# xenji/kafka-topic-analyzer

Measured on NVIDIA H100. Metric: messages/sec scanned (fused metric scan), higher is better.
Workload: dtype u64

## Files before the change

kafka_topic_analyzer_b200/csrc/kta_api.cu:

```cuda
#include <cuda_runtime.h>

#include <algorithm>
#include <chrono>
#include <climits>
#include <cmath>
#include <cstdarg>
#include <cstdio>
#include <cstdlib>
#include <cstring>
#include <new>
#include <vector>

#include "kta_host.cuh"
#include "kta_kernels.cuh"
#include "kta_logscan.cuh"
#include "kta_partitioner.cuh"
#include "kta_synth.h"
#include "kta_timeline.cuh"

using namespace kta;

extern "C" const char *kta_last_error(void) { return g_err; }
extern "C" int kta_abi_version(void) { return KTA_ABI_VERSION; }
extern "C" int kta_device_count(void) {
    int n = 0;
    if (cudaGetDeviceCount(&n) != cudaSuccess) {
        cudaGetLastError();
        return -1;
    }
    return n;
}

static constexpr int NCHUNK = 3;
static constexpr int32_t ALIVE_DEFAULT_KIB = 256 * 1024;
static constexpr int32_t ALIVE_MAX_KIB = 32 * 1024 * 1024;
static constexpr int64_t ALIVE_CACHE_MIN_RECORDS = 1 << 20;
static constexpr int64_t DEFAULT_RING_RECORDS = 1 << 22;

struct Chunk {
    DevBuf<int32_t> d_partition, d_klen, d_vlen;
    DevBuf<int64_t> d_ts;
    DevBuf<uint64_t> d_seq;
    DevBuf<uint8_t> d_keys;
    DevBuf<uint64_t> d_tile_base;
    cudaEvent_t free_ev = nullptr;
    PinnedBuf<int32_t> h_partition, h_klen, h_vlen;
    PinnedBuf<int64_t> h_ts;
    PinnedBuf<uint8_t> h_keys;
    PinnedBuf<uint64_t> h_tile_base;
};

struct AlivePending {
    ScanParams prm;
    int64_t key_readable, key_bytes;
    int chunk;
    const uint32_t *hash; const uint64_t *stamp; int64_t count;
};

struct AliveKeys {
    DevBuf<unsigned long long> d_table;
    uint32_t pairs = 0;
    uint64_t origin = 0;
    bool rebased = false;
    DevBuf<uint32_t> d_cache;
    DevBuf<uint32_t> d_status;
    PinnedBuf<uint32_t> h_status;
    DevBuf<unsigned long long> d_count;
    uint64_t window_errors = 0;
    uint64_t grows = 0, reruns = 0;
    uint64_t now = 0, occupied = 0;
    std::vector<AlivePending> pending;
};

struct Timeline {
    int32_t buckets = 0;
    int64_t origin = 0, width = 1;
    bool smem = false;
    int blocks_per_sm = 0;
    DevBuf<unsigned long long> d_bins;
    std::vector<uint64_t> h_bins;
    size_t words() const { return d_bins.cap > 0 ? (size_t)d_bins.cap : 0; }
};

struct Partitioner {
    int32_t ncounts = 0;
    int32_t counts[KTA_PARTITIONER_MAX_COUNTS] = {};
    bool smem = false;
    int32_t max_grid = 0;
    DevBuf<unsigned long long> d_counts;
    std::vector<uint64_t> h_counts;
    size_t words() const { return d_counts.cap > 0 ? (size_t)d_counts.cap : 0; }
};

struct kta_handle {
    kta_config cfg{};
    int device = 0;
    int sm_count = 0;
    cudaStream_t stream = nullptr;
    bool own_stream = true;
    bool need_hash = false;
    DevBuf<unsigned long long> d_sums;
    DevBuf<long long> d_minmax;
    DevBuf<uint32_t> d_hll;
    DevBuf<uint32_t> d_hll_floor;
    AliveKeys alive;
    uint32_t *d_hash_out = nullptr;
    DevBuf<uint64_t> d_tb_scratch;
    LogScan log;
    Timeline tl;
    Partitioner pt;
    DevBuf<uint32_t> d_crc32_tables;
    size_t nsums = 0, nhll = 0;
    Chunk chunks[NCHUNK];
    bool ring_dev_ready = false, ring_host_ready = false;
    int64_t ring_records = 0, ring_key_bytes = 0;
    int cur = 0;
    struct PushCursor {
        int32_t *part = nullptr, *klen = nullptr, *vlen = nullptr;
        int64_t *ts = nullptr;
        uint8_t *keys = nullptr;
        uint64_t *tile_base = nullptr;
        int64_t n = 0, cap = 0;
        int64_t kb = 0, kcap = 0;
        bool hash = false;
    } pc;
    uint64_t next_seq = 0;
    bool finalized = false;
    std::vector<uint64_t> h_sums;
    long long h_minmax[4] = {0, 0, 0, 0};
    std::vector<uint32_t> h_hll;
    uint64_t h_alive = 0;
    int shard_world = 1, shard_rank = 0;
    int columns = 0;
    bool smem_counters = true;
    size_t smem_optin = 0;
    uint64_t launches = 0, records = 0;
    bool timing = false;
    std::vector<std::pair<cudaEvent_t, cudaEvent_t>> ev_pool;
    size_t ev_used = 0;
    double scan_ms = 0;
    uint64_t scan_launches_timed = 0;
};

static int set_device(const kta_handle *h) {
    CU(cudaSetDevice(h->device));
    return KTA_OK;
}

static bool keys_travel(const kta_handle *h) { return h->need_hash || h->d_hash_out || h->pt.ncounts; }

static size_t scan_smem_bytes(bool hash, bool smem, int P, int threads, int keybuf, int stages, bool hdr) {
    return (smem ? smem_counter_bytes(P) : CTA_SCRATCH) + (size_t)(threads / 32) * warp_smem_bytes(hash, keybuf, stages, hdr);
}

static void scan_shape(const kta_handle *h, bool hash, bool hdr_ok, int64_t n, int64_t key_bytes, int &threads, int &keybuf,
                       int &stages, bool &hdr, size_t &smem) {
    const int P = h->columns;
    keybuf = KEYBUF_MIN;
    stages = 0;
    hdr = false;
    if (!hash) {
        threads = MAX_THREADS;
        smem = scan_smem_bytes(false, h->smem_counters, P, threads, keybuf, stages, hdr);
        return;
    }
    if (n > 0) {
        const int64_t per_tile = (key_bytes * TILE + n - 1) / n;
        int64_t want = per_tile + per_tile / 8 + 64 + KEYBUF_SLACK;
        want = (want + 127) / 128 * 128;
        keybuf = (int)std::min<int64_t>(std::max<int64_t>(want, KEYBUF_MIN), KEYBUF_MAX);
        keybuf = (keybuf + 15) / 16 * 16;
    }
    auto fits = [&](bool with_hdr, int st, int max_warps, int min_warps) {
        hdr = with_hdr;
        stages = st;
        for (threads = std::min(max_warps * 32, HASH_MAX_THREADS); threads >= min_warps * 32; threads -= 32) {
            smem = scan_smem_bytes(true, h->smem_counters, P, threads, keybuf, stages, hdr);
            if (smem <= h->smem_optin) return true;
        }
        return false;
    };
    if (hdr_ok && (fits(true, SCAN_STAGES, 12, 10) || fits(true, 2, 12, 10))) return;
    if (fits(false, 2, 16, 8)) return;
    keybuf = KEYBUF_MIN;
    fits(false, 2, 16, 1);
}

using ScanFn = void (*)(ScanParams);
static const ScanFn SCAN_KERNELS[2][2][3][2] = {
    {{{scan_kernel<MODE_COUNTERS, false, false, false>, nullptr},
      {scan_kernel<MODE_HLL, false, false, false>, scan_kernel<MODE_HLL, false, true, false>},
      {scan_kernel<MODE_EXACT, false, false, false>, scan_kernel<MODE_EXACT, false, true, false>}},
     {{scan_kernel<MODE_COUNTERS, false, false, true>, nullptr},
      {scan_kernel<MODE_HLL, false, false, true>, nullptr},
      {scan_kernel<MODE_EXACT, false, false, true>, nullptr}}},
    {{{scan_kernel<MODE_COUNTERS, true, false, false>, nullptr},
      {scan_kernel<MODE_HLL, true, false, false>, scan_kernel<MODE_HLL, true, true, false>},
      {scan_kernel<MODE_EXACT, true, false, false>, scan_kernel<MODE_EXACT, true, true, false>}},
     {{scan_kernel<MODE_COUNTERS, true, false, true>, nullptr},
      {scan_kernel<MODE_HLL, true, false, true>, nullptr},
      {scan_kernel<MODE_EXACT, true, false, true>, nullptr}}},
};

static int launch_scan_raw(kta_handle *h, ScanParams prm, int64_t key_readable, int64_t key_bytes);
static int ring_flush(kta_handle *h);

static int alive_create(kta_handle *h) {
    const int64_t kib = h->cfg.alive_table_kib;
    if (kib < 0 || kib > ALIVE_MAX_KIB) return fail(KTA_ERR_INVALID, "alive_table_kib %d out of range [0, %d]", (int)kib, ALIVE_MAX_KIB);
    AliveKeys &a = h->alive;
    a.pairs = (uint32_t)std::max<int64_t>((kib ? kib : ALIVE_DEFAULT_KIB) * 64, 16);
    int rc;
    if ((rc = a.d_table.alloc((int64_t)a.pairs * 2)) || (rc = a.d_status.alloc(3)) || (rc = a.d_count.alloc(3)) ||
        (rc = a.d_cache.alloc((int64_t)1 << ALIVE_CACHE_SET_BITS)) || (rc = a.h_status.alloc(2 * (NCHUNK + 1))))
        return rc;
    return KTA_OK;
}

static int alive_reset(kta_handle *h) {
    AliveKeys &a = h->alive;
    if (!a.d_table) return KTA_OK;
    CU(cudaMemsetAsync(a.d_table, 0xff, (size_t)a.pairs * 16, h->stream));
    CU(cudaMemsetAsync(a.d_status, 0, 12, h->stream));
    a.now = a.occupied = a.origin = 0;
    a.rebased = false;
    a.window_errors = 0;
    a.pending.clear();
    return KTA_OK;
}

static int alive_grow(kta_handle *h, uint32_t new_pairs) {
    AliveKeys &a = h->alive;
    cudaStream_t s = h->stream;
    DevBuf<unsigned long long> nt;
    int rc;
    if ((rc = nt.alloc((int64_t)new_pairs * 2))) return rc;
    CU(cudaMemsetAsync(nt, 0xff, (size_t)new_pairs * 16, s));
    alive_rehash_kernel<<<h->sm_count * 8, THREADS, 0, s>>>(a.d_table, (size_t)a.pairs * 2, nt, new_pairs, a.d_status);
    h->launches++;
    CU(cudaGetLastError());
    CU(cudaStreamSynchronize(s));
    a.d_table = std::move(nt);
    a.pairs = new_pairs;
    a.grows++;
    return KTA_OK;
}

static int alive_apply(kta_handle *h, const AlivePending &p) {
    AliveKeys &a = h->alive;
    if (p.count) {
        const int grid = (int)std::min<int64_t>((p.count + THREADS - 1) / THREADS, (int64_t)h->sm_count * 8);
        alive_import_kernel<<<grid, THREADS, 0, h->stream>>>(AliveTable{a.d_table, a.pairs, a.d_status, 0}, a.origin, p.hash,
                                                             reinterpret_cast<const unsigned long long *>(p.stamp), p.count);
        h->launches++;
        CU(cudaGetLastError());
        return KTA_OK;
    }
    ScanParams prm = p.prm;
    prm.alive_only = 1;
    prm.alive_table = a.d_table;
    prm.alive_pairs = a.pairs;
    a.reruns++;
    return launch_scan_raw(h, prm, p.key_readable, p.key_bytes);
}

static int alive_settle(kta_handle *h) {
    AliveKeys &a = h->alive;
    if (!a.d_table) return KTA_OK;
    cudaStream_t s = h->stream;
    for (int round = 0;; round++) {
        unsigned long long counts[3] = {0, 0, 0};
        CU(cudaMemsetAsync(a.d_count, 0, 24, s));
        alive_count_kernel<<<h->sm_count * 8, THREADS, 0, s>>>(a.d_table, (size_t)a.pairs * 2, a.d_count);
        h->launches++;
        CU(cudaGetLastError());
        CU(cudaMemcpyAsync(a.h_status, a.d_status, 8, cudaMemcpyDeviceToHost, s));
        CU(cudaMemcpyAsync(counts, a.d_count, 24, cudaMemcpyDeviceToHost, s));
        CU(cudaStreamSynchronize(s));
        const unsigned long long occupied = counts[2];
        a.now = counts[0];
        a.occupied = occupied;
        const uint32_t dropped = a.h_status[0];
        a.window_errors += a.h_status[1];
        if (dropped || a.h_status[1]) CU(cudaMemsetAsync(a.d_status, 0, 8, s));
        const uint64_t slots = (uint64_t)a.pairs * 2;
        const bool crowded = occupied * 10 > slots * 6;
        if (!dropped && !crowded) break;
        const bool wide = dropped && (occupied + dropped) * 10 <= slots * 6;
        int rc;
        if (!wide) {
            if (a.pairs >= (uint32_t)ALIVE_MAX_KIB * 64u) {
                if (dropped) return fail(KTA_ERR_NOMEM, "alive-key table is at its maximum (32 GiB) and still too full");
                break;
            }
            uint64_t want = slots * 2;
            while (want < (occupied + dropped) * 2) want *= 2;
            want = std::min<uint64_t>(want, (uint64_t)ALIVE_MAX_KIB * 128ull);
            if ((rc = alive_grow(h, (uint32_t)(want / 2)))) return rc;
            if (!dropped) break;
        }
        if (round > 40) return fail(KTA_ERR_INVALID, "alive-key table growth did not converge");
        if (wide) CU(cudaMemsetAsync(a.d_status + 2, 0xff, 4, s));
        for (const AlivePending &p : a.pending)
            if ((rc = alive_apply(h, p))) return rc;
        if (wide) CU(cudaMemsetAsync(a.d_status + 2, 0, 4, s));
    }
    a.pending.clear();
    return KTA_OK;
}

static int alive_settle_if_any(kta_handle *h) { return h->alive.pending.empty() ? KTA_OK : alive_settle(h); }

static int alive_prepare(kta_handle *h, ScanParams &prm, const uint64_t *seq_ends) {
    AliveKeys &a = h->alive;
    int rc;
    if ((uint64_t)prm.n > (uint64_t)ALIVE_FIELD_MAX - 1)
        return fail(KTA_ERR_INVALID, "batch of %lld records with count_alive_keys: split it (< 2^31 per scan)", (long long)prm.n);
    if (prm.seq_base < a.origin)
        return fail(KTA_ERR_INVALID, "seq_base %llu lies before the alive-key table's window origin %llu (batches must not "
                    "go back past a rebase)", (unsigned long long)prm.seq_base, (unsigned long long)a.origin);
    if (!prm.seq && prm.seq_base - a.origin + (uint64_t)prm.n > (uint64_t)ALIVE_FIELD_MAX) {
        if ((rc = alive_settle(h))) return rc;
        if (!a.pending.empty()) return fail(KTA_ERR_INVALID, "internal: alive-key stamps pending across a rebase");
        alive_rebase_kernel<<<h->sm_count * 8, THREADS, 0, h->stream>>>(a.d_table, (size_t)a.pairs * 2);
        h->launches++;
        CU(cudaGetLastError());
        a.origin = prm.seq_base;
        a.rebased = true;
    }
    prm.alive_table = a.d_table;
    prm.alive_pairs = a.pairs;
    prm.alive_origin = a.origin;
    prm.alive_fbase = prm.seq_base - a.origin + 1ull;
    prm.alive_status = a.d_status;
    if (prm.n >= ALIVE_CACHE_MIN_RECORDS) {
        uint64_t lo = prm.seq_base, hi = prm.seq_base + (uint64_t)prm.n - 1;
        bool ok = true;
        if (prm.seq) {
            uint64_t ends[2];
            if (seq_ends) { ends[0] = seq_ends[0]; ends[1] = seq_ends[1]; }
            else {
                CU(cudaMemcpyAsync(&ends[0], prm.seq, 8, cudaMemcpyDeviceToHost, h->stream));
                CU(cudaMemcpyAsync(&ends[1], prm.seq + (prm.n - 1), 8, cudaMemcpyDeviceToHost, h->stream));
                CU(cudaStreamSynchronize(h->stream));
            }
            lo = std::min(ends[0], ends[1]);
            hi = std::max(ends[0], ends[1]);
            ok = lo >= a.origin && hi - a.origin < (uint64_t)ALIVE_FIELD_MAX;
        }
        if (ok) {
            prm.alive_cache = a.d_cache;
            int sh = 0;
            while (((hi - lo) >> sh) + 1 > (uint64_t)ALIVE_CACHE_WAVES) sh++;
            prm.alive_wave_shift = sh;
            prm.alive_wave_base = (uint32_t)(lo - a.origin + 1ull);
        }
    }
    return KTA_OK;
}

static int alive_scanned(kta_handle *h, const ScanParams &prm, int64_t key_readable, int64_t key_bytes, int chunk) {
    AliveKeys &a = h->alive;
    if (chunk >= 0) CU(cudaMemcpyAsync(a.h_status + 2 * (chunk + 1), a.d_status, 8, cudaMemcpyDeviceToHost, h->stream));
    a.pending.push_back(AlivePending{prm, key_readable, key_bytes, chunk, nullptr, nullptr, 0});
    return KTA_OK;
}

static int alive_release_chunk(kta_handle *h, int ci) {
    AliveKeys &a = h->alive;
    size_t keep = a.pending.size();
    while (keep > 0 && a.pending[keep - 1].chunk != ci) keep--;
    if (keep == 0) return KTA_OK;
    const uint32_t *snap = a.h_status + 2 * (ci + 1);
    if (snap[0] | snap[1]) return alive_settle(h);
    a.pending.erase(a.pending.begin(), a.pending.begin() + (long)keep);
    return KTA_OK;
}

static int alive_export(kta_handle *h, int mode, uint32_t *dh, uint64_t *ds, int64_t cap, int64_t *count) {
    if (!h || !count) return fail(KTA_ERR_INVALID, "bad argument");
    AliveKeys &a = h->alive;
    if (!a.d_table) return fail(KTA_ERR_NOT_ENABLED, "count_alive_keys was not enabled");
    int rc;
    if ((rc = set_device(h))) return rc;
    if ((rc = ring_flush(h))) return rc;
    if ((rc = alive_settle(h))) return rc;
    if (a.rebased)
        return fail(KTA_ERR_INVALID, "the alive-key table was rebased (more than 2^31 sequence numbers since kta_reset): its "
                    "entries no longer carry absolute sequence numbers and cannot be merged across GPUs");
    CU(cudaMemsetAsync(a.d_count + 1, 0, 8, h->stream));
    alive_export_kernel<<<h->sm_count * 8, THREADS, 0, h->stream>>>(
        a.d_table, (size_t)a.pairs * 2, a.origin, mode, a.d_count + 1, dh,
        reinterpret_cast<unsigned long long *>(ds), (unsigned long long)cap);
    h->launches++;
    CU(cudaGetLastError());
    unsigned long long c = 0;
    CU(cudaMemcpyAsync(&c, a.d_count + 1, 8, cudaMemcpyDeviceToHost, h->stream));
    CU(cudaStreamSynchronize(h->stream));
    *count = (int64_t)c;
    if (mode == 1 && (int64_t)c > cap) return fail(KTA_ERR_INVALID, "export buffer too small: %llu > %lld", c, (long long)cap);
    return KTA_OK;
}

extern "C" int kta_alive_export_count(kta_handle *h, int64_t *count) { return alive_export(h, 0, nullptr, nullptr, 0, count); }

extern "C" int kta_alive_export_device(kta_handle *h, uint32_t *dev_hash, uint64_t *dev_stamp, int64_t cap, int64_t *count) {
    if (!dev_hash || !dev_stamp) return fail(KTA_ERR_INVALID, "bad argument");
    return alive_export(h, 1, dev_hash, dev_stamp, cap, count);
}

extern "C" int kta_alive_import_device(kta_handle *h, const uint32_t *dev_hash, const uint64_t *dev_stamp, int64_t count) {
    if (!h || count < 0 || (count && (!dev_hash || !dev_stamp))) return fail(KTA_ERR_INVALID, "bad argument");
    AliveKeys &a = h->alive;
    if (!a.d_table) return fail(KTA_ERR_NOT_ENABLED, "count_alive_keys was not enabled");
    if (count == 0) return KTA_OK;
    int rc;
    if ((rc = set_device(h))) return rc;
    if ((rc = alive_settle(h))) return rc;
    const AlivePending p{ScanParams{}, 0, 0, -1, dev_hash, dev_stamp, count};
    if ((rc = alive_apply(h, p))) return rc;
    a.pending.push_back(p);
    if ((rc = alive_settle(h))) return rc;
    h->finalized = false;
    return KTA_OK;
}

static int state_reset_device(kta_handle *h) {
    state_init_kernel<<<64, 256, 0, h->stream>>>(h->d_sums, h->nsums, h->d_minmax, h->d_hll, h->nhll, h->d_hll_floor);
    h->launches++;
    CU(cudaGetLastError());
    return alive_reset(h);
}

extern "C" int kta_destroy(kta_handle *h) {
    if (!h) return KTA_OK;
    cudaSetDevice(h->device);
    if (h->stream) cudaStreamSynchronize(h->stream);
    for (auto &c : h->chunks)
        if (c.free_ev) cudaEventDestroy(c.free_ev);
    for (auto &e : h->ev_pool) { cudaEventDestroy(e.first); cudaEventDestroy(e.second); }
    cudaStream_t own = h->own_stream ? h->stream : nullptr;
    delete h;
    if (own) cudaStreamDestroy(own);
    cudaGetLastError();
    return KTA_OK;
}

static int create_impl(const kta_config *cfg, kta_handle *h) {
    h->cfg = *cfg;
    if (cfg->num_partitions < 1 || cfg->num_partitions > (1 << 20))
        return fail(KTA_ERR_INVALID, "num_partitions %d out of range [1, 2^20]", cfg->num_partitions);
    if (cfg->hll_precision != 0 && (cfg->hll_precision < 4 || cfg->hll_precision > 18))
        return fail(KTA_ERR_INVALID, "hll_precision %d not 0 or 4..18", cfg->hll_precision);
    if (cfg->isolation_level != KTA_READ_UNCOMMITTED && cfg->isolation_level != KTA_READ_COMMITTED)
        return fail(KTA_ERR_INVALID, "isolation_level %d is neither KTA_READ_UNCOMMITTED (0) nor KTA_READ_COMMITTED (1)", cfg->isolation_level);
    int ndev = 0;
    CU(cudaGetDeviceCount(&ndev));
    if (ndev < 1) return fail(KTA_ERR_CUDA, "no CUDA device (this library has no CPU fallback)");
    if (cfg->device >= 0) h->device = cfg->device;
    else CU(cudaGetDevice(&h->device));
    if (h->device >= ndev) return fail(KTA_ERR_INVALID, "device %d >= device count %d", h->device, ndev);
    CU(cudaSetDevice(h->device));
    cudaDeviceProp prop;
    CU(cudaGetDeviceProperties(&prop, h->device));
    if (prop.major != 9 || prop.minor != 0) return fail(KTA_ERR_CUDA, "device %s is sm_%d%d; this library is built for sm_90a only",
                                     prop.name, prop.major, prop.minor);
    h->sm_count = prop.multiProcessorCount;
    CU(cudaStreamCreateWithFlags(&h->stream, cudaStreamNonBlocking));
    h->need_hash = cfg->count_alive_keys == 1 || cfg->hll_precision != 0;
    h->pc.hash = keys_travel(h);
    if (cfg->now_s == INT64_MIN) {
        const auto now = std::chrono::system_clock::now().time_since_epoch();
        const int64_t ns = std::chrono::duration_cast<std::chrono::nanoseconds>(now).count();
        h->cfg.now_s = ns / 1000000000ll;
        h->cfg.now_ns = (int32_t)(ns % 1000000000ll);
    }
    h->ring_records = cfg->ring_records > 0 ? cfg->ring_records : DEFAULT_RING_RECORDS;
    h->ring_records = (h->ring_records + TILE - 1) / TILE * TILE;
    h->ring_key_bytes = cfg->ring_key_bytes > 0 ? cfg->ring_key_bytes : h->ring_records * 24;

    const int P = cfg->num_partitions;
    h->nsums = sums_words(P);
    h->nhll = cfg->hll_precision ? ((size_t)1 << cfg->hll_precision) : 0;
    int rc;
    if ((rc = h->d_sums.alloc((int64_t)h->nsums)) || (rc = h->d_minmax.alloc(4)) || (rc = h->d_hll_floor.alloc(HLL_SLICES + 2)))
        return rc;
    if (h->nhll && (rc = h->d_hll.alloc((int64_t)h->nhll))) return rc;
    if (cfg->count_alive_keys == 1 && (rc = alive_create(h))) return rc;
    h->smem_optin = prop.sharedMemPerBlockOptin;
    if (cfg->shard_world > 1) {
        if (cfg->shard_rank < 0 || cfg->shard_rank >= cfg->shard_world || cfg->shard_world > P)
            return fail(KTA_ERR_INVALID, "shard_rank %d / shard_world %d invalid for %d partitions", cfg->shard_rank, cfg->shard_world, P);
        const uint64_t G = (uint64_t)cfg->shard_world, e = (((uint64_t)1 << 32) + G - 1) / G * G - ((uint64_t)1 << 32);
        if ((uint64_t)(P - 1) * e >= (uint64_t)1 << 32)
            return fail(KTA_ERR_INVALID, "shard_world %d with %d partitions: the scan's partition division is exact only when "
                        "(P - 1) * (ceil(2^32 / G) * G - 2^32) < 2^32 (every P <= 65536 and every G <= 4096 qualify)",
                        cfg->shard_world, P);
        h->shard_world = cfg->shard_world;
        h->shard_rank = cfg->shard_rank;
    }
    h->columns = (P - h->shard_rank + h->shard_world - 1) / h->shard_world;
    h->smem_counters = smem_counter_bytes(h->columns) + 8 * warp_smem_bytes(true, KEYBUF_MIN, 2, false) <= h->smem_optin;
    for (const auto &by_mode : SCAN_KERNELS[h->smem_counters])
        for (const auto &by_capture : by_mode)
            for (const ScanFn f : by_capture)
                if (f) CU(cudaFuncSetAttribute(f, cudaFuncAttributeMaxDynamicSharedMemorySize, (int)h->smem_optin));
    if ((rc = log_scan_create(h->log, cfg->isolation_level == KTA_READ_COMMITTED, h->smem_optin))) return rc;
    if ((rc = state_reset_device(h))) return rc;
    CU(cudaStreamSynchronize(h->stream));
    return KTA_OK;
}

extern "C" int kta_create(const kta_config *cfg, kta_handle **out) {
    if (!cfg || !out) return fail(KTA_ERR_INVALID, "null argument");
    if (cfg->struct_size != (int32_t)sizeof(kta_config))
        return fail(KTA_ERR_INVALID, "kta_config.struct_size %d != %zu (ABI version %d)", cfg->struct_size, sizeof(kta_config), KTA_ABI_VERSION);
    kta_handle *h = new (std::nothrow) kta_handle();
    if (!h) return fail(KTA_ERR_NOMEM, "out of host memory");
    const int rc = create_impl(cfg, h);
    if (rc) {
        char keep[sizeof(g_err)];
        memcpy(keep, g_err, sizeof(keep));
        kta_destroy(h);
        memcpy(g_err, keep, sizeof(keep));
        *out = nullptr;
        return rc;
    }
    *out = h;
    return KTA_OK;
}

extern "C" void *kta_stream(kta_handle *h) { return h ? (void *)h->stream : nullptr; }

extern "C" int kta_set_stream(kta_handle *h, void *stream) {
    if (!h) return fail(KTA_ERR_INVALID, "null handle");
    int rc;
    if ((rc = set_device(h))) return rc;
    CU(cudaStreamSynchronize(h->stream));
    if (h->own_stream) CU(cudaStreamDestroy(h->stream));
    h->stream = (cudaStream_t)stream;
    h->own_stream = false;
    return KTA_OK;
}

static int launch_scan_raw(kta_handle *h, ScanParams prm, int64_t key_readable, int64_t key_bytes) {
    const int P = h->cfg.num_partitions;
    const bool exact = h->cfg.count_alive_keys == 1;
    const bool capture = h->d_hash_out != nullptr && !prm.alive_only;
    const int mode = exact ? MODE_EXACT : (h->cfg.hll_precision || capture) ? MODE_HLL : MODE_COUNTERS;
    if (mode == MODE_HLL && !h->cfg.hll_precision)
        return fail(KTA_ERR_INVALID, "hash capture needs count_alive_keys or hll_precision");
    prm.shard_world = h->shard_world;
    prm.shard_rank = h->shard_rank;
    prm.Pc = h->columns;
    prm.shard_magic = h->shard_world > 1 ? (uint32_t)((((uint64_t)1 << 32) + (uint64_t)h->shard_world - 1) / (uint64_t)h->shard_world) : 0u;
    prm.ntiles = (prm.n + TILE - 1) / TILE;
    if (prm.ntiles >= (int64_t)1 << 30) return fail(KTA_ERR_INVALID, "batch of %lld records: split it (one scan takes < 2^37 records)", (long long)prm.n);
    prm.P = P;
    prm.hll_p = h->cfg.hll_precision;
    prm.sums = h->d_sums;
    prm.minmax = h->d_minmax;
    prm.hll = h->d_hll;
    prm.hll_floor = h->d_hll_floor;
    prm.hash_out = capture ? h->d_hash_out : nullptr;
    if (mode != MODE_COUNTERS) {
        if (!prm.key_tile_base) return fail(KTA_ERR_INVALID, "internal: key_tile_base missing");
        if (!prm.key_bytes && key_readable > 0) return fail(KTA_ERR_INVALID, "key_bytes is NULL but keys are required");
        prm.stage_limit = (((uintptr_t)prm.key_bytes & 15u) == 0) ? ((uint64_t)key_readable & ~15ull) : 0;
    }
    if (capture && h->shard_world > 1) return fail(KTA_ERR_INVALID, "hash capture is not available on a partition-sharded handle");
    int threads = 0, keybuf = 0, stages = 0;
    bool hdr = false;
    size_t sm = 0;
    const uintptr_t cols = (uintptr_t)prm.partition | (uintptr_t)prm.ts_ms | (uintptr_t)prm.key_len | (uintptr_t)prm.value_len;
    scan_shape(h, mode != MODE_COUNTERS, (cols & 15u) == 0, prm.n, key_bytes, threads, keybuf, stages, hdr, sm);
    prm.hdr_stage = hdr;
    if (sm > h->smem_optin) return fail(KTA_ERR_INVALID, "scan kernel does not fit: %zu B shared memory", sm);
    prm.keybuf = keybuf;
    prm.stages = stages;
    const int grid = (int)std::min<int64_t>((prm.ntiles + threads / 32 - 1) / (threads / 32), h->sm_count);
    if (prm.alive_cache) CU(cudaMemsetAsync(prm.alive_cache, 0, (size_t)4 << ALIVE_CACHE_SET_BITS, h->stream));
    cudaEvent_t e0 = nullptr, e1 = nullptr;
    if (h->timing) {
        if (h->ev_used == h->ev_pool.size()) {
            cudaEvent_t a, b;
            CU(cudaEventCreate(&a));
            CU(cudaEventCreate(&b));
            h->ev_pool.emplace_back(a, b);
        }
        e0 = h->ev_pool[h->ev_used].first;
        e1 = h->ev_pool[h->ev_used].second;
        h->ev_used++;
        CU(cudaEventRecord(e0, h->stream));
    }
    SCAN_KERNELS[h->smem_counters][h->shard_world > 1][mode][capture]<<<grid, threads, sm, h->stream>>>(prm);
    CU(cudaGetLastError());
    h->launches++;
    if (h->timing) CU(cudaEventRecord(e1, h->stream));
    return KTA_OK;
}

static void timeline_shape(const kta_handle *h, int64_t n, int &grid, int &threads, size_t &smem) {
    const Timeline &t = h->tl;
    const int64_t ntiles = (n + TILE - 1) / TILE;
    threads = TL_THREADS;
    smem = t.smem ? (size_t)h->cfg.num_partitions * (size_t)(t.buckets + 2) * 16 : 0;
    const int64_t warps = TL_THREADS / 32;
    int64_t g = std::min<int64_t>((ntiles + warps - 1) / warps, (int64_t)h->sm_count * t.blocks_per_sm);
    g = std::max<int64_t>(g, (ntiles + TL_MAX_CTA_TILES - 1) / TL_MAX_CTA_TILES);
    grid = (int)std::max<int64_t>(g, 1);
}

static int launch_timeline(kta_handle *h, const ScanParams &prm) {
    const Timeline &t = h->tl;
    TimelineParams tp{};
    tp.n = prm.n;
    tp.ntiles = (prm.n + TILE - 1) / TILE;
    tp.partition = prm.partition;
    tp.ts_ms = prm.ts_ms;
    tp.key_len = prm.key_len;
    tp.value_len = prm.value_len;
    tp.P = h->cfg.num_partitions;
    tp.shard_world = h->shard_world;
    tp.shard_rank = h->shard_rank;
    tp.B = t.buckets;
    tp.origin = t.origin;
    tp.width = (uint64_t)t.width;
    tp.span = (uint64_t)t.buckets * (uint64_t)t.width;
    tp.inv_width = 1.0 / (double)t.width;
    tp.out = t.d_bins;
    int grid = 0, threads = 0;
    size_t smem = 0;
    timeline_shape(h, prm.n, grid, threads, smem);
    if (t.smem) timeline_kernel<true><<<grid, threads, smem, h->stream>>>(tp);
    else timeline_kernel<false><<<grid, threads, 0, h->stream>>>(tp);
    CU(cudaGetLastError());
    h->launches++;
    return KTA_OK;
}

static int partitioner_shape(const kta_handle *h, int64_t n, int64_t key_bytes, int &grid, int &stage, size_t &smem) {
    const Partitioner &t = h->pt;
    const int64_t ntiles = (n + TILE - 1) / TILE;
    const size_t fixed = (size_t)PC_TABLE_WORDS * 4 + (t.smem ? ((size_t)(2 * t.ncounts + 1) * h->cfg.num_partitions + 3) / 4 * 16 : 0);
    const int64_t room = ((int64_t)h->smem_optin - (int64_t)fixed) / PC_WARPS - PC_STAGE_PAD;
    const int64_t per_tile = n > 0 ? (std::max<int64_t>(key_bytes, 0) * TILE + n - 1) / n : 0;
    int64_t want = (per_tile + per_tile / 8 + 64 + 15) / 16 * 16;
    want = std::min<int64_t>(std::max<int64_t>(want, PC_STAGE_MIN), PC_STAGE_MAX);
    stage = (int)std::min<int64_t>(want, room / 16 * 16);
    smem = fixed + (size_t)PC_WARPS * (size_t)(stage + PC_STAGE_PAD);
    int per_sm = 0;
    if (t.smem) CU(cudaOccupancyMaxActiveBlocksPerMultiprocessor(&per_sm, partitioner_kernel<true>, PC_THREADS, smem));
    else CU(cudaOccupancyMaxActiveBlocksPerMultiprocessor(&per_sm, partitioner_kernel<false>, PC_THREADS, smem));
    if (per_sm < 1) return fail(KTA_ERR_CUDA, "partitioner kernel does not fit an SM (%zu B shared memory)", smem);
    int64_t g = std::min<int64_t>((ntiles + PC_WARPS - 1) / PC_WARPS, (int64_t)h->sm_count * per_sm);
    if (t.max_grid) g = std::min<int64_t>(g, t.max_grid);
    g = std::max<int64_t>(g, (ntiles + PC_MAX_CTA_TILES - 1) / PC_MAX_CTA_TILES);
    grid = (int)std::max<int64_t>(g, 1);
    return KTA_OK;
}

static int launch_partitioner(kta_handle *h, const ScanParams &prm, int64_t key_bytes) {
    const Partitioner &t = h->pt;
    PartitionerParams pp{};
    pp.n = prm.n;
    pp.ntiles = (prm.n + TILE - 1) / TILE;
    pp.partition = prm.partition;
    pp.key_len = prm.key_len;
    pp.key_bytes = prm.key_bytes;
    pp.key_tile_base = prm.key_tile_base;
    pp.P = h->cfg.num_partitions;
    pp.shard_world = h->shard_world;
    pp.shard_rank = h->shard_rank;
    pp.C = t.ncounts;
    for (int j = 0; j < t.ncounts; j++) {
        pp.count[j] = (uint32_t)t.counts[j];
        pp.recip[j] = ~0ull / (uint64_t)t.counts[j] + 1ull;
    }
    pp.tables = h->d_crc32_tables;
    pp.out = t.d_counts;
    int grid = 0, rc;
    size_t smem = 0;
    if ((rc = partitioner_shape(h, prm.n, key_bytes, grid, pp.stage, smem))) return rc;
    if (t.smem) partitioner_kernel<true><<<grid, PC_THREADS, smem, h->stream>>>(pp);
    else partitioner_kernel<false><<<grid, PC_THREADS, smem, h->stream>>>(pp);
    CU(cudaGetLastError());
    h->launches++;
    return KTA_OK;
}

static int launch_scan(kta_handle *h, ScanParams prm, int64_t key_readable, int64_t key_bytes, int chunk = -1,
                       const uint64_t *seq_ends = nullptr) {
    if (prm.n <= 0) return KTA_OK;
    const bool exact = h->alive.d_table != nullptr;
    int rc;
    if (h->pt.ncounts) {
        if (!prm.key_tile_base) return fail(KTA_ERR_INVALID, "internal: key_tile_base missing");
        if (!prm.key_bytes && key_readable > 0) return fail(KTA_ERR_INVALID, "key_bytes is NULL but the partitioner check needs the keys");
    }
    if (exact && (rc = alive_prepare(h, prm, seq_ends))) return rc;
    if ((rc = launch_scan_raw(h, prm, key_readable, key_bytes))) return rc;
    if (h->tl.buckets && (rc = launch_timeline(h, prm))) return rc;
    if (h->pt.ncounts && (rc = launch_partitioner(h, prm, key_bytes))) return rc;
    if (exact && (rc = alive_scanned(h, prm, key_readable, key_bytes, chunk))) return rc;
    h->records += (uint64_t)prm.n;
    h->finalized = false;
    return KTA_OK;
}

static int collect_timing(kta_handle *h) {
    for (size_t i = 0; i < h->ev_used; i++) {
        float ms = 0;
        CU(cudaEventElapsedTime(&ms, h->ev_pool[i].first, h->ev_pool[i].second));
        h->scan_ms += ms;
        h->scan_launches_timed++;
    }
    h->ev_used = 0;
    return KTA_OK;
}

static LogEnv log_env(kta_handle *h) {
    return LogEnv{h->stream, h->sm_count, h->smem_optin, h->cfg.num_partitions, h->d_tb_scratch, h->launches};
}

static int derive_tile_base(kta_handle *h, const int32_t *d_klen, int64_t n) { return log_tile_base(log_env(h), d_klen, n); }

static ScanParams scan_params(int64_t n, uint64_t seq_base, const int32_t *partition, const int64_t *ts_ms, const int32_t *key_len,
                              const int32_t *value_len, const uint8_t *key_bytes, const uint64_t *key_tile_base, const uint64_t *seq) {
    return ScanParams{n, seq_base, partition, ts_ms, key_len, value_len, key_bytes, key_tile_base, seq};
}

static int check_batch(const kta_handle *h, const kta_batch *b) {
    if (!h || !b) return fail(KTA_ERR_INVALID, "null argument");
    if (b->n < 0) return fail(KTA_ERR_INVALID, "negative n");
    if (b->n > 0 && (!b->partition || !b->ts_ms || !b->key_len || !b->value_len))
        return fail(KTA_ERR_INVALID, "partition/ts_ms/key_len/value_len columns are required");
    return KTA_OK;
}

static int resolve_seq_base(kta_handle *h, const kta_batch *b, uint64_t *out) {
    if (b->seq_base == KTA_SEQ_AUTO) {
        *out = h->next_seq;
        return KTA_OK;
    }
    if (h->cfg.count_alive_keys == 1 && !b->seq && b->seq_base < h->next_seq)
        return fail(KTA_ERR_INVALID, "seq_base %llu < %llu, the next sequence number of this handle: batches without a seq "
                    "column must be pushed in stream order (use KTA_SEQ_AUTO to continue the running count)",
                    (unsigned long long)b->seq_base, (unsigned long long)h->next_seq);
    *out = b->seq_base;
    return KTA_OK;
}

static int scan_device_batch(kta_handle *h, const kta_batch *b) {
    uint64_t seq_base = 0;
    int rc;
    if ((rc = resolve_seq_base(h, b, &seq_base))) return rc;
    ScanParams prm = scan_params(b->n, seq_base, b->partition, b->ts_ms, b->key_len, b->value_len, b->key_bytes, b->key_tile_base, b->seq);
    if (keys_travel(h) && !prm.key_tile_base) {
        if ((rc = derive_tile_base(h, b->key_len, b->n))) return rc;
        prm.key_tile_base = h->d_tb_scratch;
    }
    if (h->pt.ncounts && !b->key_bytes) {
        if (b->key_bytes_len > 0) return fail(KTA_ERR_INVALID, "key_bytes is NULL but key_bytes_len is %lld", (long long)b->key_bytes_len);
        uint64_t total = 0;
        CU(cudaMemcpyAsync(&total, prm.key_tile_base + (b->n + TILE - 1) / TILE, 8, cudaMemcpyDeviceToHost, h->stream));
        CU(cudaStreamSynchronize(h->stream));
        if (total) return fail(KTA_ERR_INVALID, "key_bytes is NULL but the batch has %llu key bytes (the partitioner check hashes them)",
                               (unsigned long long)total);
    }
    if ((rc = launch_scan(h, prm, b->key_bytes_len, b->key_bytes_len))) return rc;
    h->next_seq = std::max<uint64_t>(h->next_seq, seq_base + (uint64_t)b->n);
    return KTA_OK;
}

extern "C" int kta_scan_batch_device(kta_handle *h, const kta_batch *b) {
    int rc;
    if ((rc = check_batch(h, b)) || b->n == 0) return rc;
    if ((rc = set_device(h))) return rc;
    if ((rc = ring_flush(h))) return rc;
    return scan_device_batch(h, b);
}


static int scan_log_batches(kta_handle *h, int32_t partition, const int32_t *dev_batch_partition, const uint8_t *dev_bytes,
                            int64_t len, int64_t readable ,
                            const uint64_t *dev_batch_off, int64_t nbatches, int64_t *records_out) {
    if (!h || len < 0 || nbatches < 0 || (nbatches && (!dev_bytes || !dev_batch_off))) return fail(KTA_ERR_INVALID, "bad argument");
    if (records_out) *records_out = 0;
    if (nbatches == 0) return KTA_OK;
    int rc;
    if ((rc = set_device(h))) return rc;
    if ((rc = ring_flush(h))) return rc;
    if ((rc = alive_settle_if_any(h))) return rc;
    LogScan &L = h->log;
    const LogEnv e = log_env(h);
    LogHeaders hd;
    if ((rc = log_headers(L, e, partition, dev_batch_partition, dev_bytes, len, dev_batch_off, nbatches, hd))) return rc;
    const int64_t ncut = hd.word.cut;
    uint64_t nrec = hd.nrec, dropped = 0;
    if (hd.nrec > 0) {
        const uint32_t codecs = hd.word.flags & LOGB_CODECS;
        if (codecs) {
            uint64_t unc_total = 0;
            uint32_t bad = 0;
            if ((rc = log_unc_size(L, e, dev_bytes, nbatches, codecs, &unc_total, &bad))) return rc;
            if (bad) return fail(KTA_ERR_INVALID, "malformed compressed record batch in partition %d", partition);
            if ((rc = log_unc_copy(L, e, dev_bytes, nbatches, codecs, unc_total))) return rc;
        }
        if (ncut && (rc = log_cut_count(L, e, dev_bytes, nbatches, ncut, &nrec, &dropped))) return rc;
        const bool keys = nrec > 0 && keys_travel(h);
        kta_batch b;
        if ((rc = log_decode(L, e, dev_bytes, readable, nbatches, nrec, hd.word.longest, keys, ncut, b))) return rc;
        if ((rc = log_gather_keys(L, e, partition, dev_bytes, keys, b))) return rc;
        if (nrec > 0 && (rc = scan_device_batch(h, &b))) return rc;
    }
    for (int i = 0; i < 3; i++) L.txn.totals[i] += hd.txn_stats[i];
    const uint32_t not_served = hd.word.not_served;
    OffsetState &o = L.offsets;
    o.totals[0] += not_served;
    o.totals[1] += hd.word.not_served_records + dropped;
    CrcState &c = L.crc;
    if (c.on) {
        c.totals[0] += (uint64_t)nbatches - not_served;
        c.totals[1] += hd.word.crc_failed;
        c.totals[2] += hd.word.crc_failed_bytes;
        c.kept.insert(c.kept.end(), hd.crc_fails.begin(), hd.crc_fails.end());
    }
    if (records_out) *records_out = (int64_t)nrec;
    return KTA_OK;
}

extern "C" int kta_scan_log_segment_device(kta_handle *h, int32_t partition, const uint8_t *dev_bytes, int64_t len,
                                           const uint64_t *dev_batch_off, int64_t nbatches, int64_t *records_out) {
    return scan_log_batches(h, partition, nullptr, dev_bytes, len, len, dev_batch_off, nbatches, records_out);
}

extern "C" int kta_scan_log_batches_device(kta_handle *h, const uint8_t *dev_bytes, int64_t len, const uint64_t *dev_batch_off,
                                           const int32_t *dev_batch_partition, int64_t nbatches, int64_t *records_out) {
    if (nbatches && !dev_batch_partition) return fail(KTA_ERR_INVALID, "dev_batch_partition is NULL");
    return scan_log_batches(h, 0, dev_batch_partition, dev_bytes, len, len, dev_batch_off, nbatches, records_out);
}

extern "C" int kta_push_log_segments_host(kta_handle *h, int32_t nsegs, const int32_t *partitions, const uint8_t *const *bytes,
                                          const int64_t *lens, int64_t *records_out) {
    if (!h || nsegs < 0 || (nsegs && (!partitions || !bytes || !lens))) return fail(KTA_ERR_INVALID, "bad argument");
    if (records_out) *records_out = 0;
    std::vector<uint64_t> offs;
    std::vector<int32_t> parts;
    std::vector<int64_t> used((size_t)nsegs, 0), base((size_t)nsegs, 0);
    int64_t total = 0;
    for (int32_t sgi = 0; sgi < nsegs; sgi++) {
        if (lens[sgi] < 0 || (lens[sgi] && !bytes[sgi])) return fail(KTA_ERR_INVALID, "bad segment %d", sgi);
        base[(size_t)sgi] = total;
        const int64_t pos = log_walk_batches(bytes[sgi], lens[sgi], total, offs);
        parts.resize(offs.size(), partitions[sgi]);
        used[(size_t)sgi] = pos;
        total += (pos + 15) & ~(int64_t)15;
    }
    if (offs.empty()) return KTA_OK;
    int rc;
    if ((rc = set_device(h))) return rc;
    cudaStream_t s = h->stream;
    LogScan &L = h->log;
    const int64_t nb = (int64_t)offs.size();
    if ((rc = L.bytes.grow(s, total + 64)) || (rc = L.off.grow(s, nb)) || (rc = L.part.grow(s, nb))) return rc;
    for (int32_t sgi = 0; sgi < nsegs; sgi++)
        if (used[(size_t)sgi])
            CU(cudaMemcpyAsync(L.bytes + base[(size_t)sgi], bytes[sgi], (size_t)used[(size_t)sgi], cudaMemcpyHostToDevice, s));
    CU(cudaMemcpyAsync(L.off, offs.data(), offs.size() * 8, cudaMemcpyHostToDevice, s));
    CU(cudaMemcpyAsync(L.part, parts.data(), parts.size() * 4, cudaMemcpyHostToDevice, s));
    if ((rc = scan_log_batches(h, 0, L.part, L.bytes, total, total + 48, L.off, nb, records_out))) return rc;
    CU(cudaStreamSynchronize(s));
    return collect_timing(h);
}

extern "C" int kta_push_log_segment_host(kta_handle *h, int32_t partition, const uint8_t *bytes, int64_t len,
                                         int64_t *records_out) {
    return kta_push_log_segments_host(h, 1, &partition, &bytes, &len, records_out);
}

extern "C" int kta_log_add_txn_index_host(kta_handle *h, int32_t partition, const uint8_t *bytes, int64_t len) {
    if (!h || len < 0 || (len && !bytes)) return fail(KTA_ERR_INVALID, "bad argument");
    if (!h->log.read_committed) return fail(KTA_ERR_INVALID, "transaction index on a read_uncommitted handle");
    if (partition < 0 || partition >= h->cfg.num_partitions)
        return fail(KTA_ERR_INVALID, "partition %d outside [0, %d)", partition, h->cfg.num_partitions);
    constexpr int64_t ENTRY = 34;
    if (len % ENTRY) return fail(KTA_ERR_INVALID, "transaction index of %lld bytes: not a multiple of %lld", (long long)len, (long long)ENTRY);
    auto be = [](const uint8_t *p, int n) { uint64_t v = 0; for (int i = 0; i < n; i++) v = (v << 8) | p[i]; return v; };
    std::vector<TxnRange> add;
    for (int64_t at = 0; at < len; at += ENTRY) {
        const uint8_t *e = bytes + at;
        const TxnRange r{partition, 0u, be(e + 2, 8), (int64_t)be(e + 10, 8), (int64_t)be(e + 18, 8)};
        if (be(e, 2) != 0) return fail(KTA_ERR_INVALID, "transaction index entry %lld: version %d", (long long)(at / ENTRY), (int)be(e, 2));
        if (r.first > r.last)
            return fail(KTA_ERR_INVALID, "transaction index entry %lld: firstOffset %lld > lastOffset %lld", (long long)(at / ENTRY),
                        (long long)r.first, (long long)r.last);
        add.push_back(r);
    }
    if (add.empty()) return KTA_OK;
    int rc;
    if ((rc = set_device(h))) return rc;
    return log_add_txn_ranges(h->log, log_env(h), add);
}

extern "C" int kta_log_txn_stats(kta_handle *h, uint64_t *aborted_batches, uint64_t *aborted_records, uint64_t *undecided_records) {
    if (!h) return fail(KTA_ERR_INVALID, "null handle");
    if (!h->log.read_committed) return fail(KTA_ERR_NOT_ENABLED, "the handle is read_uncommitted");
    if (aborted_batches) *aborted_batches = h->log.txn.totals[0];
    if (aborted_records) *aborted_records = h->log.txn.totals[1];
    if (undecided_records) *undecided_records = h->log.txn.totals[2];
    return KTA_OK;
}

extern "C" int kta_log_set_check_crcs(kta_handle *h, int enabled) {
    if (!h) return fail(KTA_ERR_INVALID, "null handle");
    if (enabled != 0 && enabled != 1) return fail(KTA_ERR_INVALID, "check_crcs %d is neither 0 nor 1", enabled);
    h->log.crc.on = enabled == 1;
    return KTA_OK;
}

extern "C" int kta_log_crc_stats(kta_handle *h, uint64_t *checked_batches, uint64_t *failed_batches, uint64_t *failed_bytes) {
    if (!h) return fail(KTA_ERR_INVALID, "null handle");
    if (checked_batches) *checked_batches = h->log.crc.totals[0];
    if (failed_batches) *failed_batches = h->log.crc.totals[1];
    if (failed_bytes) *failed_bytes = h->log.crc.totals[2];
    return KTA_OK;
}

extern "C" int kta_log_set_offsets(kta_handle *h, int32_t partition, int64_t log_start_offset, int64_t high_watermark) {
    if (!h) return fail(KTA_ERR_INVALID, "null handle");
    if (partition < 0 || partition >= h->cfg.num_partitions)
        return fail(KTA_ERR_INVALID, "partition %d outside [0, %d)", partition, h->cfg.num_partitions);
    if (log_start_offset < -1 || high_watermark < -1)
        return fail(KTA_ERR_INVALID, "log start offset %lld / high watermark %lld below -1", (long long)log_start_offset,
                    (long long)high_watermark);
    if (log_start_offset >= 0 && high_watermark >= 0 && log_start_offset > high_watermark)
        return fail(KTA_ERR_INVALID, "log start offset %lld above the high watermark %lld", (long long)log_start_offset,
                    (long long)high_watermark);
    log_set_window(h->log, h->cfg.num_partitions, partition, log_start_offset, high_watermark);
    return KTA_OK;
}

extern "C" int kta_log_offset_stats(kta_handle *h, uint64_t *batches_not_served, uint64_t *records_left_out) {
    if (!h) return fail(KTA_ERR_INVALID, "null handle");
    if (batches_not_served) *batches_not_served = h->log.offsets.totals[0];
    if (records_left_out) *records_left_out = h->log.offsets.totals[1];
    return KTA_OK;
}

extern "C" int kta_log_crc_failures(kta_handle *h, kta_log_crc_failure *out, int64_t cap, int64_t *count) {
    if (!h || cap < 0 || (cap && !out)) return fail(KTA_ERR_INVALID, "bad argument");
    const std::vector<kta_log_crc_failure> &kept = h->log.crc.kept;
    const size_t n = std::min<size_t>((size_t)cap, kept.size());
    if (n) memcpy(out, kept.data(), n * sizeof(kta_log_crc_failure));
    if (count) *count = (int64_t)kept.size();
    return KTA_OK;
}

static int ring_dev_init(kta_handle *h) {
    if (h->ring_dev_ready) return KTA_OK;
    const int64_t R = h->ring_records, KB = h->ring_key_bytes;
    int rc;
    for (auto &c : h->chunks) {
        if ((rc = c.d_partition.alloc(R)) || (rc = c.d_klen.alloc(R)) || (rc = c.d_vlen.alloc(R)) || (rc = c.d_ts.alloc(R)) ||
            (rc = c.d_seq.alloc(R)) || (rc = c.d_keys.alloc(KB + 64)) || (rc = c.d_tile_base.alloc(R / TILE + 2)))
            return rc;
        if (!c.free_ev) CU(cudaEventCreateWithFlags(&c.free_ev, cudaEventDisableTiming));
    }
    h->ring_dev_ready = true;
    return KTA_OK;
}

static int ring_host_init(kta_handle *h) {
    if (h->ring_host_ready) return KTA_OK;
    int rc;
    if ((rc = ring_dev_init(h))) return rc;
    const int64_t R = h->ring_records, KB = h->ring_key_bytes;
    for (auto &c : h->chunks)
        if ((rc = c.h_partition.alloc(R)) || (rc = c.h_klen.alloc(R)) || (rc = c.h_vlen.alloc(R)) || (rc = c.h_ts.alloc(R)) ||
            (rc = c.h_keys.alloc(KB + 64)) || (rc = c.h_tile_base.alloc(R / TILE + 2)))
            return rc;
    h->ring_host_ready = true;
    return KTA_OK;
}

static void push_cursor_bind(kta_handle *h) {
    Chunk &c = h->chunks[h->cur];
    auto &pc = h->pc;
    pc.part = c.h_partition; pc.klen = c.h_klen; pc.vlen = c.h_vlen; pc.ts = c.h_ts; pc.keys = c.h_keys; pc.tile_base = c.h_tile_base;
    pc.n = 0; pc.kb = 0;
    pc.cap = h->ring_host_ready ? h->ring_records : 0;
    pc.kcap = h->ring_key_bytes;
    pc.hash = keys_travel(h);
}

static int ring_scan_chunk(kta_handle *h, const ScanParams &prm, int64_t key_readable, int64_t key_bytes,
                           const uint64_t *seq_ends = nullptr) {
    int rc;
    if ((rc = launch_scan(h, prm, key_readable, key_bytes, h->cur, seq_ends))) return rc;
    CU(cudaEventRecord(h->chunks[h->cur].free_ev, h->stream));
    h->cur = (h->cur + 1) % NCHUNK;
    return KTA_OK;
}

static int ring_reuse_chunk(kta_handle *h, int ci) {
    CU(cudaEventSynchronize(h->chunks[ci].free_ev));
    return alive_release_chunk(h, ci);
}

static int ring_flush(kta_handle *h) {
    if (h->pc.n == 0) return KTA_OK;
    Chunk &c = h->chunks[h->cur];
    const int64_t n = h->pc.n, kb = h->pc.kb;
    const int64_t ntiles = (n + TILE - 1) / TILE;
    c.h_tile_base[ntiles] = (uint64_t)kb;
    cudaStream_t s = h->stream;
    CU(cudaMemcpyAsync(c.d_partition, c.h_partition, n * 4, cudaMemcpyHostToDevice, s));
    CU(cudaMemcpyAsync(c.d_ts, c.h_ts, n * 8, cudaMemcpyHostToDevice, s));
    CU(cudaMemcpyAsync(c.d_klen, c.h_klen, n * 4, cudaMemcpyHostToDevice, s));
    CU(cudaMemcpyAsync(c.d_vlen, c.h_vlen, n * 4, cudaMemcpyHostToDevice, s));
    if (keys_travel(h)) {
        if (kb) CU(cudaMemcpyAsync(c.d_keys, c.h_keys, kb, cudaMemcpyHostToDevice, s));
        CU(cudaMemcpyAsync(c.d_tile_base, c.h_tile_base, (ntiles + 1) * 8, cudaMemcpyHostToDevice, s));
    }
    const ScanParams prm = scan_params(n, h->next_seq, c.d_partition, c.d_ts, c.d_klen, c.d_vlen, c.d_keys, c.d_tile_base, nullptr);
    int rc;
    if ((rc = ring_scan_chunk(h, prm, (kb + 15) & ~(int64_t)15, kb))) return rc;
    h->next_seq += (uint64_t)n;
    push_cursor_bind(h);
    return ring_reuse_chunk(h, h->cur);
}

static int __attribute__((noinline)) push_slow(kta_handle *h, int64_t kl) {
    int rc;
    if ((rc = set_device(h))) return rc;
    if (!h->ring_host_ready) {
        if ((rc = ring_host_init(h))) return rc;
        push_cursor_bind(h);
    }
    if (kl > h->ring_key_bytes) return fail(KTA_ERR_INVALID, "key of %lld bytes exceeds ring_key_bytes", (long long)kl);
    if (h->pc.n == h->pc.cap || h->pc.kb + kl > h->pc.kcap) return ring_flush(h);
    return KTA_OK;
}

extern "C" int kta_push(kta_handle *h, int32_t partition, int64_t offset, int64_t ts_ms, const uint8_t *key,
                        int32_t key_len, int32_t value_len) {
    (void)offset;
    if (__builtin_expect(!h, 0)) return fail(KTA_ERR_INVALID, "null handle");
    auto &pc = h->pc;
    const int64_t kl = (pc.hash && key_len > 0) ? key_len : 0;
    if (__builtin_expect(pc.n == pc.cap || pc.kb + kl > pc.kcap, 0)) {
        const int rc = push_slow(h, kl);
        if (rc) return rc;
    }
    const int64_t i = pc.n;
    if ((i & (TILE - 1)) == 0) pc.tile_base[i / TILE] = (uint64_t)pc.kb;
    pc.part[i] = partition;
    pc.ts[i] = ts_ms;
    pc.klen[i] = key_len < 0 ? -1 : key_len;
    pc.vlen[i] = value_len < 0 ? -1 : value_len;
    if (kl) {
        if (__builtin_expect(!key, 0)) return fail(KTA_ERR_INVALID, "key is NULL with key_len %d", key_len);
        uint8_t *dst = pc.keys + pc.kb;
        if (kl == 16) {
            uint64_t a, b;
            memcpy(&a, key, 8); memcpy(&b, key + 8, 8);
            memcpy(dst, &a, 8); memcpy(dst + 8, &b, 8);
        } else if (kl <= 8) {
            for (int64_t j = 0; j < kl; j++) dst[j] = key[j];
        } else {
            memcpy(dst, key, (size_t)kl);
        }
        pc.kb += kl;
    }
    pc.n = i + 1;
    h->finalized = false;
    return KTA_OK;
}

extern "C" int kta_push_batch_host(kta_handle *h, const kta_batch *b) {
    int rc;
    if ((rc = check_batch(h, b)) || b->n == 0) return rc;
    const bool hash = keys_travel(h);
    if (hash && !b->key_bytes && b->key_bytes_len > 0) return fail(KTA_ERR_INVALID, "key_bytes is NULL");
    if (h->pt.ncounts && !b->key_bytes)
        for (int64_t i = 0; i < b->n; i++)
            if (b->key_len[i] > 0) return fail(KTA_ERR_INVALID, "key_bytes is NULL but record %lld has a %d-byte key (the partitioner "
                                               "check hashes it)", (long long)i, b->key_len[i]);
    if ((rc = set_device(h))) return rc;
    if ((rc = ring_flush(h))) return rc;
    if ((rc = ring_dev_init(h))) return rc;
    uint64_t seq_base = 0;
    if ((rc = resolve_seq_base(h, b, &seq_base))) return rc;
    cudaStream_t s = h->stream;
    const bool use_seq = b->seq && h->cfg.count_alive_keys == 1;
    std::vector<uint64_t> tb_host;
    uint64_t koff = 0;
    int64_t r0 = 0;
    while (r0 < b->n) {
        int64_t cn = std::min<int64_t>(h->ring_records, b->n - r0);
        const int ci = h->cur;
        Chunk &c = h->chunks[ci];
        uint64_t k0 = 0, k1 = 0;
        const uint64_t *tb_src = nullptr;
        if (hash) {
            const int64_t tiles_max = (cn + TILE - 1) / TILE;
            int64_t tiles = 0;
            if (b->key_tile_base) {
                const uint64_t *tb = b->key_tile_base + r0 / TILE;
                k0 = tb[0];
                tiles = std::upper_bound(tb, tb + tiles_max + 1, k0 + (uint64_t)h->ring_key_bytes) - tb - 1;
                tiles = std::min<int64_t>(tiles, tiles_max);
                if (tiles >= 1) k1 = tb[tiles];
                tb_src = tb;
            } else {
                tb_host.resize((size_t)tiles_max + 1);
                uint64_t acc = koff;
                tb_host[0] = acc;
                for (; tiles < tiles_max; tiles++) {
                    const int64_t lo = r0 + tiles * TILE, hi = std::min<int64_t>(lo + TILE, r0 + cn);
                    uint64_t tile_bytes = 0;
                    for (int64_t i = lo; i < hi; i++) tile_bytes += b->key_len[i] > 0 ? (uint64_t)b->key_len[i] : 0;
                    if (acc + tile_bytes - koff > (uint64_t)h->ring_key_bytes) break;
                    acc += tile_bytes;
                    tb_host[(size_t)tiles + 1] = acc;
                }
                k0 = koff;
                k1 = acc;
                tb_src = tb_host.data();
            }
            if (tiles < 1)
                return fail(KTA_ERR_INVALID, "the keys of one %d-record tile (records %lld..) exceed ring_key_bytes %lld; "
                            "%lld earlier record(s) of this batch were scanned", TILE, (long long)r0, (long long)h->ring_key_bytes,
                            (long long)r0);
            cn = std::min<int64_t>(cn, tiles * TILE);
        }
        if ((rc = ring_reuse_chunk(h, ci))) return rc;
        const int64_t ntiles = (cn + TILE - 1) / TILE;
        CU(cudaMemcpyAsync(c.d_partition, b->partition + r0, cn * 4, cudaMemcpyHostToDevice, s));
        CU(cudaMemcpyAsync(c.d_ts, b->ts_ms + r0, cn * 8, cudaMemcpyHostToDevice, s));
        CU(cudaMemcpyAsync(c.d_klen, b->key_len + r0, cn * 4, cudaMemcpyHostToDevice, s));
        CU(cudaMemcpyAsync(c.d_vlen, b->value_len + r0, cn * 4, cudaMemcpyHostToDevice, s));
        if (use_seq) CU(cudaMemcpyAsync(c.d_seq, b->seq + r0, cn * 8, cudaMemcpyHostToDevice, s));
        const uint64_t shift = k0 & 15ull;
        if (hash) {
            if (k1 > k0) CU(cudaMemcpyAsync(c.d_keys + shift, b->key_bytes + k0, k1 - k0, cudaMemcpyHostToDevice, s));
            CU(cudaMemcpyAsync(c.d_tile_base, tb_src, (ntiles + 1) * 8, cudaMemcpyHostToDevice, s));
        }
        const ScanParams prm = scan_params(cn, seq_base + (uint64_t)r0, c.d_partition, c.d_ts, c.d_klen, c.d_vlen,
                                           hash ? c.d_keys + shift - k0 : nullptr, hash ? c.d_tile_base.get() : nullptr,
                                           use_seq ? c.d_seq.get() : nullptr);
        const uint64_t seq_ends[2] = {use_seq ? b->seq[r0] : 0, use_seq ? b->seq[r0 + cn - 1] : 0};
        if ((rc = ring_scan_chunk(h, prm, (int64_t)((k1 + 15) & ~15ull), (int64_t)(k1 - k0), use_seq ? seq_ends : nullptr))) return rc;
        koff = k1;
        r0 += cn;
    }
    CU(cudaStreamSynchronize(s));
    if ((rc = collect_timing(h))) return rc;
    h->next_seq = std::max<uint64_t>(h->next_seq, seq_base + (uint64_t)b->n);
    return KTA_OK;
}

extern "C" int kta_sync(kta_handle *h) {
    if (!h) return fail(KTA_ERR_INVALID, "null handle");
    int rc;
    if ((rc = set_device(h))) return rc;
    if ((rc = ring_flush(h))) return rc;
    CU(cudaStreamSynchronize(h->stream));
    if ((rc = alive_settle(h))) return rc;
    return collect_timing(h);
}

extern "C" int kta_reset(kta_handle *h) {
    if (!h) return fail(KTA_ERR_INVALID, "null handle");
    int rc;
    if ((rc = set_device(h))) return rc;
    h->pc.n = 0;
    h->pc.kb = 0;
    h->next_seq = 0;
    h->finalized = false;
    h->launches = 0;
    h->records = 0;
    h->log.txn.ranges.clear();
    for (uint64_t &v : h->log.txn.totals) v = 0;
    for (uint64_t &v : h->log.crc.totals) v = 0;
    h->log.crc.kept.clear();
    OffsetState &o = h->log.offsets;
    std::fill(o.win.begin(), o.win.end(), make_longlong2(-1, -1));
    o.set = 0;
    o.dirty = !o.win.empty();
    for (uint64_t &v : o.totals) v = 0;
    if (h->tl.buckets) CU(cudaMemsetAsync(h->tl.d_bins, 0, h->tl.words() * 8, h->stream));
    if (h->pt.ncounts) CU(cudaMemsetAsync(h->pt.d_counts, 0, h->pt.words() * 8, h->stream));
    return state_reset_device(h);
}

extern "C" int kta_finalize(kta_handle *h) {
    if (!h) return fail(KTA_ERR_INVALID, "null handle");
    int rc;
    if ((rc = set_device(h))) return rc;
    if ((rc = ring_flush(h))) return rc;
    cudaStream_t s = h->stream;
    if ((rc = alive_settle(h))) return rc;
    if (h->alive.d_table && h->nhll) {
        CU(cudaMemsetAsync(h->d_hll, 0, h->nhll * 4, s));
        alive_hll_kernel<<<h->sm_count * 8, THREADS, 0, s>>>(h->alive.d_table, (size_t)h->alive.pairs * 2, h->d_hll,
                                                             h->cfg.hll_precision);
        CU(cudaGetLastError());
        h->launches++;
    }
    h->h_sums.resize(h->nsums);
    h->h_hll.resize(h->nhll);
    CU(cudaMemcpyAsync(h->h_sums.data(), h->d_sums, h->nsums * 8, cudaMemcpyDeviceToHost, s));
    CU(cudaMemcpyAsync(h->h_minmax, h->d_minmax, 32, cudaMemcpyDeviceToHost, s));
    if (h->nhll) CU(cudaMemcpyAsync(h->h_hll.data(), h->d_hll, h->nhll * 4, cudaMemcpyDeviceToHost, s));
    if (h->tl.buckets) {
        h->tl.h_bins.resize(h->tl.words());
        CU(cudaMemcpyAsync(h->tl.h_bins.data(), h->tl.d_bins, h->tl.words() * 8, cudaMemcpyDeviceToHost, s));
    }
    if (h->pt.ncounts) {
        h->pt.h_counts.resize(h->pt.words());
        CU(cudaMemcpyAsync(h->pt.h_counts.data(), h->pt.d_counts, h->pt.words() * 8, cudaMemcpyDeviceToHost, s));
    }
    CU(cudaStreamSynchronize(s));
    if ((rc = collect_timing(h))) return rc;
    h->h_alive = h->alive.now;
    h->finalized = true;
    if (h->alive.window_errors)
        return fail(KTA_ERR_INVALID, "%llu record(s) carried a sequence number outside the alive-key table's window "
                    "[origin, origin + 2^31 - 2): with an explicit seq column the span between kta_reset calls is limited",
                    (unsigned long long)h->alive.window_errors);
    const uint64_t bad = h->h_sums[h->nsums - 1];
    if (bad)
        return fail(KTA_ERR_PARTITION, "%llu record(s) had a partition outside [0, %d) and were left out of every metric",
                    (unsigned long long)bad, h->cfg.num_partitions);
    return KTA_OK;
}

static int check_read(const kta_handle *h, int32_t p, bool per_partition) {
    if (!h) return fail(KTA_ERR_INVALID, "null handle");
    if (!h->finalized) return fail(KTA_ERR_NOT_FINALIZED, "call kta_finalize first");
    if (per_partition && (p < 0 || p >= h->cfg.num_partitions)) return -1;
    return KTA_OK;
}

static uint64_t raw_counter(const kta_handle *h, int which, int32_t p) {
    const int P = h->cfg.num_partitions;
    const uint64_t *s = h->h_sums.data();
    uint64_t knn = 0, alive = 0;
    for (int b = 0; b < NB; b++) {
        knn += s[(size_t)p * NB + b];
        alive += s[(size_t)(P + p) * NB + b];
    }
    const uint64_t knull = s[(size_t)P * (2 * NB + 2) + p];
    const uint64_t total = knn + knull;
    switch (which) {
        case KTA_TOTAL: return total;
        case KTA_TOMBSTONES: return total - alive;
        case KTA_ALIVE: return alive;
        case KTA_KEY_NULL: return knull;
        case KTA_KEY_NON_NULL: return knn;
        case KTA_KEY_SIZE_SUM: return s[(size_t)P * (2 * NB) + p];
        case KTA_VALUE_SIZE_SUM: return s[(size_t)P * (2 * NB + 1) + p];
    }
    return 0;
}

extern "C" int kta_counter(const kta_handle *h, int which, int32_t partition, uint64_t *out) {
    if (!out || which < 0 || which > KTA_VALUE_SIZE_SUM) return fail(KTA_ERR_INVALID, "bad argument");
    const int rc = check_read(h, partition, true);
    if (rc > 0) return rc;
    *out = rc < 0 ? 0 : raw_counter(h, which, partition);
    return KTA_OK;
}

extern "C" int kta_avg(const kta_handle *h, int which, int32_t partition, uint64_t *out) {
    if (!out || which < 0 || which > KTA_MESSAGE_SIZE_AVG) return fail(KTA_ERR_INVALID, "bad argument");
    const int rc = check_read(h, partition, true);
    if (rc > 0) return rc;
    if (rc < 0) { *out = 0; return KTA_OK; }
    const uint64_t ks = raw_counter(h, KTA_KEY_SIZE_SUM, partition), vs = raw_counter(h, KTA_VALUE_SIZE_SUM, partition);
    const uint64_t alive = raw_counter(h, KTA_ALIVE, partition);
    const uint64_t sum = which == KTA_KEY_SIZE_AVG ? ks : which == KTA_VALUE_SIZE_AVG ? vs : ks + vs;
    if (sum > 0) {
        if (alive == 0)
            return fail(KTA_ERR_DIV_BY_ZERO, "partition %d: sum %llu > 0 with alive == 0 (the reference panics here)",
                        partition, (unsigned long long)sum);
        *out = sum / alive;
    } else {
        *out = 0;
    }
    return KTA_OK;
}

extern "C" int kta_dirty_ratio(const kta_handle *h, int32_t partition, float *out) {
    if (!out) return fail(KTA_ERR_INVALID, "bad argument");
    const int rc = check_read(h, partition, true);
    if (rc > 0) return rc;
    *out = 0.0f;
    if (rc < 0) return KTA_OK;
    const uint64_t total = raw_counter(h, KTA_TOTAL, partition), tomb = raw_counter(h, KTA_TOMBSTONES, partition);
    if (total > 0 && tomb > 0) {
        const volatile float t = (float)tomb;
        const volatile float d = (float)total / 100.0f;
        *out = t / d;
    }
    return KTA_OK;
}

extern "C" int kta_global(const kta_handle *h, int which, uint64_t *out) {
    if (!out) return fail(KTA_ERR_INVALID, "bad argument");
    const int rc = check_read(h, 0, false);
    if (rc) return rc;
    const int P = h->cfg.num_partitions;
    const unsigned long long *mm = reinterpret_cast<const unsigned long long *>(h->h_minmax);
    switch (which) {
        case KTA_SMALLEST_MESSAGE: *out = mm[2] == ~0ull ? 0 : mm[2]; return KTA_OK;
        case KTA_LARGEST_MESSAGE: *out = mm[3]; return KTA_OK;
        case KTA_OVERALL_SIZE: {
            uint64_t s = 0;
            for (int p = 0; p < P; p++) s += raw_counter(h, KTA_KEY_SIZE_SUM, p) + raw_counter(h, KTA_VALUE_SIZE_SUM, p);
            *out = s;
            return KTA_OK;
        }
        case KTA_OVERALL_COUNT: {
            uint64_t s = 0;
            for (int p = 0; p < P; p++) s += raw_counter(h, KTA_TOTAL, p);
            *out = s;
            return KTA_OK;
        }
    }
    return fail(KTA_ERR_INVALID, "bad global id %d", which);
}

extern "C" int kta_timestamps(const kta_handle *h, int64_t *earliest_s, int32_t *earliest_ns, int64_t *latest_s) {
    const int rc = check_read(h, 0, false);
    if (rc) return rc;
    int64_t es = h->cfg.now_s, ls = 0;
    int32_t ens = h->cfg.now_ns;
    if (h->h_minmax[0] != INT64_MAX) {
        const int64_t raw_mn = h->h_minmax[0] == -1 ? 0 : h->h_minmax[0];
        const int64_t raw_mx = h->h_minmax[1] == -1 ? 0 : h->h_minmax[1];
        const int64_t mn = raw_mn / 1000, mx = raw_mx / 1000;
        if (es > mn || (es == mn && ens > 0)) { es = mn; ens = 0; }
        if (ls < mx) ls = mx;
    }
    if (earliest_s) *earliest_s = es;
    if (earliest_ns) *earliest_ns = ens;
    if (latest_s) *latest_s = ls;
    return KTA_OK;
}

extern "C" int kta_alive_keys(const kta_handle *h, uint64_t *out) {
    if (!out) return fail(KTA_ERR_INVALID, "bad argument");
    const int rc = check_read(h, 0, false);
    if (rc) return rc;
    if (h->cfg.count_alive_keys != 1) return fail(KTA_ERR_NOT_ENABLED, "count_alive_keys was not enabled");
    *out = h->h_alive;
    return KTA_OK;
}

extern "C" int kta_bad_partition_records(const kta_handle *h, uint64_t *out) {
    if (!out) return fail(KTA_ERR_INVALID, "bad argument");
    const int rc = check_read(h, 0, false);
    if (rc) return rc;
    *out = h->h_sums[h->nsums - 1];
    return KTA_OK;
}

extern "C" int kta_hist(const kta_handle *h, int which, int32_t partition, uint64_t out[KTA_HIST_BUCKETS]) {
    if (!out || which < 0 || which > 1) return fail(KTA_ERR_INVALID, "bad argument");
    const int rc = check_read(h, partition, true);
    if (rc > 0) return rc;
    const int P = h->cfg.num_partitions;
    for (int b = 0; b < NB; b++)
        out[b] = rc < 0 ? 0 : h->h_sums[(size_t)((which ? P : 0) + partition) * NB + b];
    return KTA_OK;
}

extern "C" int kta_set_timeline(kta_handle *h, int64_t origin_s, int64_t width_s, int32_t buckets) {
    if (!h) return fail(KTA_ERR_INVALID, "null handle");
    if (h->records || h->pc.n)
        return fail(KTA_ERR_INVALID, "the timeline is configured before the first record: records were pushed or scanned "
                    "since create or the last kta_reset");
    if (width_s < 1) return fail(KTA_ERR_INVALID, "timeline width %lld s: must be at least 1", (long long)width_s);
    if (buckets < 0 || buckets > TL_MAX_BUCKETS)
        return fail(KTA_ERR_INVALID, "timeline buckets %d outside [0, %d]", buckets, TL_MAX_BUCKETS);
    __int128 end = (__int128)origin_s + (__int128)buckets * (__int128)width_s;
    if (end > (__int128)INT64_MAX)
        return fail(KTA_ERR_INVALID, "timeline origin %lld + %d buckets x %lld s overflows int64", (long long)origin_s, buckets,
                    (long long)width_s);
    const int64_t P = h->cfg.num_partitions;
    const int64_t bins = P * ((int64_t)buckets + 2);
    if (buckets && bins > TL_MAX_BINS)
        return fail(KTA_ERR_INVALID, "timeline of %lld partitions x %d indices exceeds 2^24 bins", (long long)P, buckets + 2);
    int rc;
    if ((rc = set_device(h))) return rc;
    Timeline t;
    if (buckets) {
        if ((rc = t.d_bins.alloc(3 * bins))) return rc;
        t.buckets = buckets;
        t.origin = origin_s;
        t.width = width_s;
        t.smem = (size_t)bins * 16 <= h->smem_optin;
        if (t.smem) {
            CU(cudaFuncSetAttribute(timeline_kernel<true>, cudaFuncAttributeMaxDynamicSharedMemorySize, (int)h->smem_optin));
            CU(cudaOccupancyMaxActiveBlocksPerMultiprocessor(&t.blocks_per_sm, timeline_kernel<true>, TL_THREADS, (size_t)bins * 16));
        } else {
            CU(cudaOccupancyMaxActiveBlocksPerMultiprocessor(&t.blocks_per_sm, timeline_kernel<false>, TL_THREADS, 0));
        }
        if (t.blocks_per_sm < 1) return fail(KTA_ERR_CUDA, "timeline kernel does not fit an SM");
        CU(cudaMemsetAsync(t.d_bins, 0, (size_t)t.d_bins.cap * 8, h->stream));
        t.h_bins.assign((size_t)t.d_bins.cap, 0);
    }
    CU(cudaStreamSynchronize(h->stream));
    h->tl = std::move(t);
    return KTA_OK;
}

extern "C" int kta_timeline(const kta_handle *h, int which, int32_t partition, uint64_t *out, int64_t cap) {
    if (!h || which < KTA_TIMELINE_RECORDS || which > KTA_TIMELINE_BYTES || cap < 0 || (cap && !out))
        return fail(KTA_ERR_INVALID, "bad argument");
    if (!h->tl.buckets) return fail(KTA_ERR_NOT_ENABLED, "the timeline is off (kta_set_timeline)");
    const int rc = check_read(h, partition, true);
    if (rc > 0) return rc;
    const int64_t row = (int64_t)h->tl.buckets + 2, n = std::min<int64_t>(cap, row);
    if (rc < 0) {
        std::fill(out, out + n, (uint64_t)0);
        return KTA_OK;
    }
    const size_t at = ((size_t)which * (size_t)h->cfg.num_partitions + (size_t)partition) * (size_t)row;
    std::copy(h->tl.h_bins.begin() + (long)at, h->tl.h_bins.begin() + (long)(at + (size_t)n), out);
    return KTA_OK;
}

extern "C" int kta_timeline_shape(const kta_handle *h, int64_t n, int32_t *grid, int32_t *threads, int32_t *smem_bins) {
    if (!h || n < 0 || !grid || !threads || !smem_bins) return fail(KTA_ERR_INVALID, "bad argument");
    if (!h->tl.buckets) return fail(KTA_ERR_NOT_ENABLED, "the timeline is off (kta_set_timeline)");
    int g = 0, th = 0;
    size_t sm = 0;
    timeline_shape(h, n, g, th, sm);
    *grid = g;
    *threads = th;
    *smem_bins = h->tl.smem ? 1 : 0;
    return KTA_OK;
}

extern "C" int kta_set_partitioner_check(kta_handle *h, const int32_t *counts, int32_t ncounts) {
    if (!h) return fail(KTA_ERR_INVALID, "null handle");
    if (h->records || h->pc.n)
        return fail(KTA_ERR_INVALID, "the partitioner check is configured before the first record: records were pushed or "
                    "scanned since create or the last kta_reset");
    if (ncounts < 0 || ncounts > KTA_PARTITIONER_MAX_COUNTS)
        return fail(KTA_ERR_INVALID, "partitioner check of %d counts: outside [0, %d]", ncounts, KTA_PARTITIONER_MAX_COUNTS);
    if (ncounts && !counts) return fail(KTA_ERR_INVALID, "counts is NULL");
    for (int j = 0; j < ncounts; j++) {
        if (counts[j] < 1) return fail(KTA_ERR_INVALID, "partition count %d: outside [1, 2^31 - 1]", counts[j]);
        for (int i = 0; i < j; i++)
            if (counts[i] == counts[j]) return fail(KTA_ERR_INVALID, "partition count %d given twice", counts[j]);
    }
    int rc;
    if ((rc = set_device(h))) return rc;
    if (ncounts && !h->d_crc32_tables) {
        uint32_t tables[4][256];
        crc_slicing_tables_host(tables, ZLIB_CRC32_POLY);
        DevBuf<uint32_t> d;
        if ((rc = d.alloc(PC_TABLE_WORDS))) return rc;
        CU(cudaMemcpy(d, &tables[0][0], sizeof tables, cudaMemcpyHostToDevice));
        h->d_crc32_tables = std::move(d);
    }
    Partitioner t;
    if (ncounts) {
        const int64_t words = (int64_t)(2 * ncounts + 1) * h->cfg.num_partitions;
        if ((rc = t.d_counts.alloc(words))) return rc;
        t.ncounts = ncounts;
        std::copy(counts, counts + ncounts, t.counts);
        t.smem = (size_t)PC_TABLE_WORDS * 4 + (size_t)(words + 3) / 4 * 16 + (size_t)PC_WARPS * (PC_STAGE_MIN + PC_STAGE_PAD) <= h->smem_optin;
        CU(cudaFuncSetAttribute(partitioner_kernel<true>, cudaFuncAttributeMaxDynamicSharedMemorySize, (int)h->smem_optin));
        CU(cudaFuncSetAttribute(partitioner_kernel<false>, cudaFuncAttributeMaxDynamicSharedMemorySize, (int)h->smem_optin));
        CU(cudaMemsetAsync(t.d_counts, 0, (size_t)words * 8, h->stream));
        t.h_counts.assign((size_t)words, 0);
    }
    CU(cudaStreamSynchronize(h->stream));
    h->pt = std::move(t);
    h->pc.hash = keys_travel(h);
    return KTA_OK;
}

extern "C" int kta_partitioner_check(const kta_handle *h, int32_t partition, uint64_t *out, int64_t cap) {
    if (!h || cap < 0 || (cap && !out)) return fail(KTA_ERR_INVALID, "bad argument");
    if (!h->pt.ncounts) return fail(KTA_ERR_NOT_ENABLED, "the partitioner check is off (kta_set_partitioner_check)");
    const int rc = check_read(h, partition, true);
    if (rc > 0) return rc;
    const int64_t nv = 2 * (int64_t)h->pt.ncounts + 1, n = std::min<int64_t>(cap, nv);
    for (int64_t b = 0; b < n; b++)
        out[b] = rc < 0 ? 0 : h->pt.h_counts[(size_t)b * (size_t)h->cfg.num_partitions + (size_t)partition];
    return KTA_OK;
}

extern "C" int kta_partitioner_shape(const kta_handle *h, int64_t n, int64_t key_bytes, int32_t *grid, int32_t *stage,
                                     int32_t *smem_counters) {
    if (!h || n < 0 || !grid || !stage || !smem_counters) return fail(KTA_ERR_INVALID, "bad argument");
    if (!h->pt.ncounts) return fail(KTA_ERR_NOT_ENABLED, "the partitioner check is off (kta_set_partitioner_check)");
    int rc;
    if ((rc = set_device(h))) return rc;
    int g = 0, st = 0;
    size_t sm = 0;
    if ((rc = partitioner_shape(h, n, key_bytes, g, st, sm))) return rc;
    *grid = g;
    *stage = st;
    *smem_counters = h->pt.smem ? 1 : 0;
    return KTA_OK;
}

extern "C" int kta_partitioner_limit_grid(kta_handle *h, int32_t max_ctas) {
    if (!h || max_ctas < 0) return fail(KTA_ERR_INVALID, "bad argument");
    if (!h->pt.ncounts) return fail(KTA_ERR_NOT_ENABLED, "the partitioner check is off (kta_set_partitioner_check)");
    h->pt.max_grid = max_ctas;
    return KTA_OK;
}

static double hll_sigma(double x) {
    if (x == 1.0) return INFINITY;
    double y = 1.0, z = x, zo;
    do { x *= x; zo = z; z += x * y; y += y; } while (zo != z);
    return z;
}
static double hll_tau(double x) {
    if (x == 0.0 || x == 1.0) return 0.0;
    double y = 1.0, z = 1.0 - x, zo;
    do { x = std::sqrt(x); zo = z; y *= 0.5; z -= (1.0 - x) * (1.0 - x) * y; } while (zo != z);
    return z / 3.0;
}

extern "C" int kta_alive_keys_hll(const kta_handle *h, double *out) {
    if (!out) return fail(KTA_ERR_INVALID, "bad argument");
    const int rc = check_read(h, 0, false);
    if (rc) return rc;
    if (!h->nhll) return fail(KTA_ERR_NOT_ENABLED, "hll_precision was 0");
    const int p = h->cfg.hll_precision, q = 32 - p;
    const double m = (double)h->nhll;
    std::vector<double> C((size_t)q + 2, 0.0);
    for (uint32_t r : h->h_hll) C[std::min<uint32_t>(r, (uint32_t)q + 1)] += 1.0;
    double z = m * hll_tau(1.0 - C[(size_t)q + 1] / m);
    for (int k = q; k >= 1; k--) z = 0.5 * (z + C[(size_t)k]);
    z += m * hll_sigma(C[0] / m);
    *out = 0.72134752044448170368 * m * m / z;
    return KTA_OK;
}

extern "C" int kta_hll_registers(const kta_handle *h, uint8_t *out, size_t cap) {
    if (!out) return fail(KTA_ERR_INVALID, "bad argument");
    const int rc = check_read(h, 0, false);
    if (rc) return rc;
    if (!h->nhll) return fail(KTA_ERR_NOT_ENABLED, "hll_precision was 0");
    if (cap < h->nhll) return fail(KTA_ERR_INVALID, "buffer too small: %zu < %zu", cap, h->nhll);
    for (size_t i = 0; i < h->nhll; i++) out[i] = (uint8_t)h->h_hll[i];
    return KTA_OK;
}

extern "C" int kta_fnv32_host(kta_handle *h, int64_t n, const int32_t *key_len, const uint8_t *key_bytes,
                              int64_t key_bytes_len, uint32_t *out) {
    if (!h || n < 0 || (n && (!key_len || !out))) return fail(KTA_ERR_INVALID, "bad argument");
    if (n == 0) return KTA_OK;
    int rc;
    if ((rc = set_device(h))) return rc;
    std::vector<uint64_t> off((size_t)n);
    uint64_t acc = 0;
    for (int64_t i = 0; i < n; i++) {
        off[(size_t)i] = acc;
        acc += key_len[i] > 0 ? (uint64_t)key_len[i] : 0;
    }
    if ((int64_t)acc > key_bytes_len) return fail(KTA_ERR_INVALID, "key_bytes_len %lld < sum of key_len %llu",
                                                  (long long)key_bytes_len, (unsigned long long)acc);
    DevBuf<int32_t> d_len;
    DevBuf<uint64_t> d_off;
    DevBuf<uint8_t> d_keys;
    DevBuf<uint32_t> d_out;
    cudaStream_t s = h->stream;
    if ((rc = d_len.alloc(n)) || (rc = d_off.alloc(n)) || (rc = d_keys.alloc((int64_t)acc + 16)) || (rc = d_out.alloc(n))) return rc;
    CU(cudaMemcpyAsync(d_len, key_len, n * 4, cudaMemcpyHostToDevice, s));
    CU(cudaMemcpyAsync(d_off, off.data(), n * 8, cudaMemcpyHostToDevice, s));
    if (acc) CU(cudaMemcpyAsync(d_keys, key_bytes, acc, cudaMemcpyHostToDevice, s));
    fnv32_kernel<<<(int)std::min<int64_t>((n + 255) / 256, 1024), 256, 0, s>>>(n, d_len, d_off, d_keys, d_out);
    h->launches++;
    CU(cudaGetLastError());
    CU(cudaMemcpyAsync(out, d_out, n * 4, cudaMemcpyDeviceToHost, s));
    CU(cudaStreamSynchronize(s));
    return KTA_OK;
}

extern "C" int kta_partitioner_hash_host(kta_handle *h, int64_t n, const int32_t *key_len, const uint8_t *key_bytes,
                                         int64_t key_bytes_len, uint32_t *murmur2, uint32_t *crc32) {
    if (!h || n < 0 || (n && (!key_len || !murmur2 || !crc32))) return fail(KTA_ERR_INVALID, "bad argument");
    if (n == 0) return KTA_OK;
    int rc;
    if ((rc = set_device(h))) return rc;
    std::vector<uint64_t> off((size_t)n);
    uint64_t acc = 0;
    for (int64_t i = 0; i < n; i++) {
        off[(size_t)i] = acc;
        acc += key_len[i] > 0 ? (uint64_t)key_len[i] : 0;
    }
    if ((int64_t)acc > key_bytes_len) return fail(KTA_ERR_INVALID, "key_bytes_len %lld < sum of key_len %llu",
                                                  (long long)key_bytes_len, (unsigned long long)acc);
    if (acc && !key_bytes) return fail(KTA_ERR_INVALID, "key_bytes is NULL");
    uint32_t tables[4][256];
    crc_slicing_tables_host(tables, ZLIB_CRC32_POLY);
    DevBuf<int32_t> d_len;
    DevBuf<uint64_t> d_off;
    DevBuf<uint8_t> d_keys;
    DevBuf<uint32_t> d_out, d_tables;
    cudaStream_t s = h->stream;
    if ((rc = d_len.alloc(n)) || (rc = d_off.alloc(n)) || (rc = d_keys.alloc((int64_t)acc + 16)) || (rc = d_out.alloc(2 * n)) ||
        (rc = d_tables.alloc(PC_TABLE_WORDS)))
        return rc;
    CU(cudaMemcpyAsync(d_len, key_len, n * 4, cudaMemcpyHostToDevice, s));
    CU(cudaMemcpyAsync(d_off, off.data(), n * 8, cudaMemcpyHostToDevice, s));
    CU(cudaMemcpyAsync(d_tables, &tables[0][0], sizeof tables, cudaMemcpyHostToDevice, s));
    if (acc) CU(cudaMemcpyAsync(d_keys, key_bytes, acc, cudaMemcpyHostToDevice, s));
    partitioner_hash_kernel<<<(int)std::min<int64_t>((n + 255) / 256, 1024), 256, 0, s>>>(n, d_len, d_off, d_keys, d_tables, d_out,
                                                                                         d_out + n);
    h->launches++;
    CU(cudaGetLastError());
    CU(cudaMemcpyAsync(murmur2, d_out, n * 4, cudaMemcpyDeviceToHost, s));
    CU(cudaMemcpyAsync(crc32, d_out + n, n * 4, cudaMemcpyDeviceToHost, s));
    CU(cudaStreamSynchronize(s));
    return KTA_OK;
}

extern "C" int kta_set_hash_capture(kta_handle *h, uint32_t *dev_out) {
    if (!h) return fail(KTA_ERR_INVALID, "null handle");
    int rc;
    if ((rc = set_device(h))) return rc;
    if ((rc = ring_flush(h))) return rc;
    h->d_hash_out = dev_out;
    h->pc.hash = keys_travel(h);
    return KTA_OK;
}

static size_t merge_base_words(const kta_handle *h, int32_t world) { return h->nsums + (size_t)world * 4 + (size_t)world * (h->nhll / 8); }

extern "C" int64_t kta_merge_words(const kta_handle *h, int32_t world) {
    if (!h || world < 1) return -1;
    return (int64_t)(merge_base_words(h, world) + h->tl.words() + h->pt.words());
}

extern "C" int kta_merge_export_device(kta_handle *h, int32_t rank, int32_t world, uint64_t *dev_buf) {
    if (!h || !dev_buf || world < 1 || rank < 0 || rank >= world) return fail(KTA_ERR_INVALID, "bad argument");
    int rc;
    if ((rc = set_device(h))) return rc;
    if ((rc = ring_flush(h))) return rc;
    if ((rc = alive_settle_if_any(h))) return rc;
    merge_export_kernel<<<h->sm_count, 256, 0, h->stream>>>(h->d_sums, h->nsums, h->d_minmax, h->d_hll, h->nhll, rank,
                                                           world, reinterpret_cast<unsigned long long *>(dev_buf));
    h->launches++;
    CU(cudaGetLastError());
    if (h->tl.buckets)
        CU(cudaMemcpyAsync(dev_buf + merge_base_words(h, world), h->tl.d_bins, h->tl.words() * 8, cudaMemcpyDeviceToDevice, h->stream));
    if (h->pt.ncounts)
        CU(cudaMemcpyAsync(dev_buf + merge_base_words(h, world) + h->tl.words(), h->pt.d_counts, h->pt.words() * 8,
                           cudaMemcpyDeviceToDevice, h->stream));
    if (h->own_stream) {
        CU(cudaStreamSynchronize(h->stream));
        return collect_timing(h);
    }
    return KTA_OK;
}

extern "C" int kta_merge_import_device(kta_handle *h, int32_t world, const uint64_t *dev_buf) {
    if (!h || !dev_buf || world < 1) return fail(KTA_ERR_INVALID, "bad argument");
    int rc;
    if ((rc = set_device(h))) return rc;
    merge_import_kernel<<<h->sm_count, 256, 0, h->stream>>>(h->d_sums, h->nsums, h->d_minmax, h->d_hll, h->nhll,
                                                           h->d_hll_floor, world,
                                                           reinterpret_cast<const unsigned long long *>(dev_buf));
    h->launches++;
    CU(cudaGetLastError());
    if (h->tl.buckets)
        CU(cudaMemcpyAsync(h->tl.d_bins, dev_buf + merge_base_words(h, world), h->tl.words() * 8, cudaMemcpyDeviceToDevice, h->stream));
    if (h->pt.ncounts)
        CU(cudaMemcpyAsync(h->pt.d_counts, dev_buf + merge_base_words(h, world) + h->tl.words(), h->pt.words() * 8,
                           cudaMemcpyDeviceToDevice, h->stream));
    h->finalized = false;
    if (h->own_stream) CU(cudaStreamSynchronize(h->stream));
    return KTA_OK;
}

extern "C" int kta_stats(const kta_handle *h, uint64_t *kernel_launches, uint64_t *records_scanned) {
    if (!h) return fail(KTA_ERR_INVALID, "null handle");
    if (kernel_launches) *kernel_launches = h->launches;
    if (records_scanned) *records_scanned = h->records;
    return KTA_OK;
}

extern "C" int kta_alive_table_stats(kta_handle *h, uint64_t *slots, uint64_t *occupied, uint64_t *grows, uint64_t *reruns) {
    if (!h) return fail(KTA_ERR_INVALID, "null handle");
    if (!h->alive.d_table) return fail(KTA_ERR_NOT_ENABLED, "count_alive_keys was not enabled");
    int rc;
    if ((rc = set_device(h))) return rc;
    if ((rc = ring_flush(h))) return rc;
    if ((rc = alive_settle(h))) return rc;
    if (slots) *slots = (uint64_t)h->alive.pairs * 2;
    if (occupied) *occupied = h->alive.occupied;
    if (grows) *grows = h->alive.grows;
    if (reruns) *reruns = h->alive.reruns;
    return KTA_OK;
}

extern "C" int kta_set_timing(kta_handle *h, int enabled) {
    if (!h) return fail(KTA_ERR_INVALID, "null handle");
    h->timing = enabled != 0;
    h->scan_ms = 0;
    h->scan_launches_timed = 0;
    return KTA_OK;
}

extern "C" int kta_scan_time_ms(kta_handle *h, double *total_ms, uint64_t *launches) {
    if (!h) return fail(KTA_ERR_INVALID, "null handle");
    int rc;
    if ((rc = set_device(h))) return rc;
    CU(cudaStreamSynchronize(h->stream));
    if ((rc = collect_timing(h))) return rc;
    if (total_ms) *total_ms = h->scan_ms;
    if (launches) *launches = h->scan_launches_timed;
    return KTA_OK;
}
```

kafka_topic_analyzer_b200/csrc/kta_kernels.cuh:

```cuda
#pragma once
#include <cuda_runtime.h>
#include <stdint.h>

#include <type_traits>

#include "../../include/kta.h"

namespace kta {

constexpr int MAX_THREADS = 1024;
constexpr int HASH_MAX_THREADS = 512;
constexpr int TILE = KTA_KEY_TILE;
constexpr int ROWS = TILE / 32;
constexpr int NB = KTA_HIST_BUCKETS;
constexpr int KEYBUF_MIN = TILE * 18 + 32, KEYBUF_MAX = TILE * 128 + 32, KEYBUF_SLACK = 32;
constexpr int HDR_P = 0, HDR_TS = TILE * 4, HDR_KL = TILE * 12, HDR_VL = TILE * 16;
constexpr int HDR_BYTES = TILE * 20;
constexpr int SCAN_STAGES = 3;
constexpr int MAX_STAGES = 4;
static_assert(SCAN_STAGES >= 2 && SCAN_STAGES <= MAX_STAGES, "2..4 stages per warp");
__host__ __device__ inline size_t warp_smem_bytes(bool hash, int keybuf, int stages, bool hdr) {
    return hash ? 128 + (size_t)stages * ((size_t)keybuf + (hdr ? HDR_BYTES : 0)) : 128;
}
constexpr uint32_t FNV_BASIS = 0x811c9dc5u;
constexpr uint32_t FNV_MULT = 0x811c9dc5u;
constexpr int FOLD_TILES = 8;

constexpr int ROW_V = NB + 1, ROW_KSUM = 2 * NB + 2, ROW_VSUM = 2 * NB + 4, SMEM_ROWS = 2 * NB + 6;
enum ScanMode { MODE_COUNTERS = 0, MODE_HLL = 1, MODE_EXACT = 2 };

__host__ __device__ inline size_t sums_words(int P) { return (size_t)P * (2 * NB + 3) + 1; }
constexpr int CTA_SCRATCH = 128;
__host__ __device__ inline size_t smem_counter_bytes(int P) { return (((size_t)P * SMEM_ROWS * 4 + 127) & ~(size_t)127) + CTA_SCRATCH; }

struct ScanParams {
    int64_t n;
    uint64_t seq_base;
    const int32_t *partition;
    const int64_t *ts_ms;
    const int32_t *key_len;
    const int32_t *value_len;
    const uint8_t *key_bytes;
    const uint64_t *key_tile_base;
    const uint64_t *seq;
    int64_t ntiles;
    int32_t P;
    int32_t shard_world, shard_rank;
    int32_t Pc;
    uint32_t shard_magic;
    int32_t hll_p;
    uint64_t stage_limit;
    int32_t hdr_stage;
    int32_t keybuf;
    int32_t stages;
    int32_t pad0;
    unsigned long long *sums;
    long long *minmax;
    uint32_t *hll;
    uint32_t *hll_floor;
    unsigned long long *alive_table;
    uint32_t alive_pairs;
    int32_t alive_only;
    uint64_t alive_origin;
    uint64_t alive_fbase;
    uint32_t *alive_cache;
    int32_t alive_wave_shift;
    uint32_t alive_wave_base;
    uint32_t *alive_status;
    uint32_t *hash_out;
};

__device__ __forceinline__ uint32_t smem_u32(const void *p) {
    uint32_t a;
    asm volatile("{ .reg .u64 t; cvta.to.shared.u64 t, %1; cvt.u32.u64 %0, t; }" : "=r"(a) : "l"(p));
    return a;
}

__device__ __forceinline__ void mbar_init(uint32_t bar, uint32_t count) {
    asm volatile("mbarrier.init.shared::cta.b64 [%0], %1;" ::"r"(bar), "r"(count));
}
__device__ __forceinline__ void fence_mbar_init() {
    asm volatile("fence.mbarrier_init.release.cluster;" ::: "memory");
}
__device__ __forceinline__ void mbar_arrive_expect_tx(uint32_t bar, uint32_t bytes) {
    asm volatile("mbarrier.arrive.expect_tx.shared::cta.b64 _, [%0], %1;" ::"r"(bar), "r"(bytes) : "memory");
}
__device__ __forceinline__ void mbar_wait(uint32_t bar, uint32_t parity) {
    asm volatile(
        "{\n\t.reg .pred p;\n\t"
        "KTA_WAIT_%=:\n\t"
        "mbarrier.try_wait.parity.shared::cta.b64 p, [%0], %1;\n\t"
        "@p bra KTA_DONE_%=;\n\t"
        "bra KTA_WAIT_%=;\n\t"
        "KTA_DONE_%=:\n\t}"
        ::"r"(bar), "r"(parity)
        : "memory");
}
__device__ __forceinline__ void bulk_g2s(uint32_t dst_smem, const void *src_gmem, uint32_t bytes, uint32_t bar) {
    asm volatile(
        "cp.async.bulk.shared::cluster.global.mbarrier::complete_tx::bytes [%0], [%1], %2, [%3];"
        ::"r"(dst_smem), "l"(src_gmem), "r"(bytes), "r"(bar)
        : "memory");
}
__device__ __forceinline__ void bulk_g2s(uint32_t dst_smem, const void *src_gmem, uint32_t bytes, uint32_t bar, uint64_t pol) {
    asm volatile(
        "cp.async.bulk.shared::cluster.global.mbarrier::complete_tx::bytes.L2::cache_hint [%0], [%1], %2, [%3], %4;"
        ::"r"(dst_smem), "l"(src_gmem), "r"(bytes), "r"(bar), "l"(pol)
        : "memory");
}
__device__ __forceinline__ void red_shared_add(uint32_t addr, uint32_t v) {
    asm volatile("red.shared.add.u32 [%0], %1;" ::"r"(addr), "r"(v) : "memory");
}
__device__ __forceinline__ uint32_t hi32(long long v) {
    uint32_t hi;
    asm("{ .reg .b32 lo; mov.b64 {lo, %0}, %1; }" : "=r"(hi) : "l"(v));
    return hi;
}
__device__ __forceinline__ long long pack64(uint32_t lo, uint32_t hi) {
    long long v;
    asm("mov.b64 %0, {%1, %2};" : "=l"(v) : "r"(lo), "r"(hi));
    return v;
}
__device__ __forceinline__ void red_shared_add_nz(uint32_t addr, uint32_t v) {
    asm volatile("{ .reg .pred p; setp.ne.u32 p, %1, 0; @p red.shared.add.u32 [%0], %1; }" ::"r"(addr), "r"(v) : "memory");
}
__device__ __forceinline__ uint4 lds128(uint32_t addr) {
    uint4 v;
    asm volatile("ld.shared.v4.u32 {%0, %1, %2, %3}, [%4];" : "=r"(v.x), "=r"(v.y), "=r"(v.z), "=r"(v.w) : "r"(addr));
    return v;
}
__device__ __forceinline__ uint32_t lds32(uint32_t addr) {
    uint32_t v;
    asm volatile("ld.shared.u32 %0, [%1];" : "=r"(v) : "r"(addr));
    return v;
}
__device__ __forceinline__ long long lds64(uint32_t addr) {
    long long v;
    asm volatile("ld.shared.s64 %0, [%1];" : "=l"(v) : "r"(addr));
    return v;
}
__device__ __forceinline__ uint32_t bfind_u32(uint32_t x) {
    uint32_t r;
    asm("bfind.u32 %0, %1;" : "=r"(r) : "r"(x));
    return r;
}
__device__ __forceinline__ int32_t ld_stream_s32(const int32_t *p) {
    int32_t v;
    asm volatile("ld.global.nc.L1::no_allocate.s32 %0, [%1];" : "=r"(v) : "l"(p));
    return v;
}
__device__ __forceinline__ int64_t ld_stream_s64(const int64_t *p) {
    int64_t v;
    asm volatile("ld.global.nc.L1::no_allocate.s64 %0, [%1];" : "=l"(v) : "l"(p));
    return v;
}
__device__ __forceinline__ uint64_t ld_stream_u64(const uint64_t *p) {
    uint64_t v;
    asm volatile("ld.global.nc.L1::no_allocate.u64 %0, [%1];" : "=l"(v) : "l"(p));
    return v;
}
__device__ __forceinline__ int32_t ld_stream_s32(const int32_t *p, uint64_t pol) {
    int32_t v;
    asm volatile("ld.global.nc.L1::no_allocate.L2::cache_hint.s32 %0, [%1], %2;" : "=r"(v) : "l"(p), "l"(pol));
    return v;
}
__device__ __forceinline__ int64_t ld_stream_s64(const int64_t *p, uint64_t pol) {
    int64_t v;
    asm volatile("ld.global.nc.L1::no_allocate.L2::cache_hint.s64 %0, [%1], %2;" : "=l"(v) : "l"(p), "l"(pol));
    return v;
}
__device__ __forceinline__ uint32_t ld_cg_u32(const uint32_t *p) {
    uint32_t v;
    asm volatile("ld.global.cg.u32 %0, [%1];" : "=r"(v) : "l"(p));
    return v;
}
__device__ __forceinline__ void red_global_max(uint32_t *p, uint32_t v) {
    asm volatile("red.global.max.u32 [%0], %1;" ::"l"(p), "r"(v) : "memory");
}

__device__ __forceinline__ uint32_t fnv_step(uint32_t h, uint32_t byte) { return (h ^ byte) * FNV_MULT; }

__device__ __forceinline__ uint32_t shr_fma(uint32_t w, uint32_t two_pow_32_minus_s) {
    uint32_t r;
    asm("mul.hi.u32 %0, %1, %2;" : "=r"(r) : "r"(w), "r"(two_pow_32_minus_s));
    return r;
}

__device__ __forceinline__ uint32_t fnv_word(uint32_t h, uint32_t w) {
    h = fnv_step(h, w & 0xffu);
    h = fnv_step(h, shr_fma(w, 1u << 24) & 0xffu);
    h = fnv_step(h, shr_fma(w, 1u << 16) & 0xffu);
    h = fnv_step(h, shr_fma(w, 1u << 8));
    return h;
}

__device__ __forceinline__ uint32_t fnv_smem(uint32_t buf_addr, uint32_t a, int len) {
    uint32_t h = FNV_BASIS;
    const uint32_t wp = buf_addr + (a & ~3u);
    const uint32_t sh = (a & 3u) * 8u;
    uint32_t lo = lds32(wp);
    int j = 0;
    for (; j + 4 <= len; j += 4) {
        const uint32_t hi = lds32(wp + j + 4);
        h = fnv_word(h, __funnelshift_r(lo, hi, sh));
        lo = hi;
    }
    const int rem = len - j;
    if (rem > 0) {
        const uint32_t hi = lds32(wp + j + 4);
        uint32_t w = __funnelshift_r(lo, hi, sh);
        for (int r = 0; r < rem; r++) {
            h = fnv_step(h, w & 0xffu);
            w >>= 8;
        }
    }
    return h;
}

__device__ __forceinline__ uint32_t fnv_global(const uint8_t *key, int len) {
    uint32_t h = FNV_BASIS;
    for (int j = 0; j < len; j++) h = fnv_step(h, (uint32_t)__ldg(key + j));
    return h;
}

__host__ __device__ __forceinline__ uint32_t hll_mix(uint32_t h) {
#ifdef __CUDA_ARCH__
    h ^= shr_fma(h, 1u << 16);
    h *= 0x85ebca6bu;
    h ^= shr_fma(h, 1u << 19);
    h *= 0xc2b2ae35u;
    h ^= shr_fma(h, 1u << 16);
    return h;
#else
    h ^= h >> 16;
    h *= 0x85ebca6bu;
    h ^= h >> 13;
    h *= 0xc2b2ae35u;
    h ^= h >> 16;
    return h;
#endif
}

__host__ __device__ __forceinline__ uint32_t hll_unmix(uint32_t h) {
    h ^= h >> 16;
    h *= 0x7ed1b41du;
    h ^= (h >> 13) ^ (h >> 26);
    h *= 0xa5cb9243u;
    h ^= h >> 16;
    return h;
}

__device__ __forceinline__ uint32_t hll_skip_mask(int p, uint32_t floor) {
    const uint32_t f = min(floor, (uint32_t)(32 - p));
    return f ? (((1u << f) - 1u) << (32 - p - f)) : 0u;
}

__device__ __forceinline__ void hll_raise(uint32_t *regs, int p, uint32_t x) {
    const uint32_t rest = x << p;
    const uint32_t rho = min((uint32_t)__clz((int)rest) + 1u, (uint32_t)(32 - p + 1));
    red_global_max(regs + (x >> (32 - p)), rho);
}

__device__ __forceinline__ void hll_update(uint32_t *regs, int p, uint32_t skip_mask, uint32_t hash) {
    const uint32_t x = hll_mix(hash);
    if ((x & skip_mask) == 0) hll_raise(regs, p, x);
}

constexpr int HLL_SLICES = 64;
__device__ __noinline__ void hll_refresh_slice(const uint32_t *regs, int p, uint32_t *aux, uint32_t slice, int lane) {
    const uint32_t n = 1u << p;
    const uint32_t per = n >= HLL_SLICES ? n / HLL_SLICES : n;
    const uint32_t base = n >= HLL_SLICES ? slice * per : 0u;
    uint32_t m = 255;
    for (uint32_t i = lane; i < per; i += 32) m = min(m, ld_cg_u32(regs + base + i));
    m = __reduce_min_sync(0xffffffffu, m);
    if (lane == 0 && m) atomicMax(aux + 1 + slice, m);
    uint32_t f;
    {
        const uint32_t s0 = (uint32_t)lane, s1 = (uint32_t)lane + 32u;
        const uint32_t v0 = s0 == slice ? m : ld_cg_u32(aux + 1 + s0);
        const uint32_t v1 = s1 == slice ? m : ld_cg_u32(aux + 1 + s1);
        f = min(v0, v1);
    }
    f = __reduce_min_sync(0xffffffffu, f);
    if (lane == 0 && f) atomicMax(aux, f);
}

template <bool SMEM>
struct Counters {
    uint32_t sbase;
    uint32_t *s;
    unsigned long long *g;
    int P;
    int Pg, G, R;
    __device__ __forceinline__ int part(int c) const { return c * G + R; }
    __device__ __forceinline__ void row_add(int r, int p, uint32_t c) const {
        if (SMEM) red_shared_add(sbase + 4u * (uint32_t)(r * P + p), c);
        else if (r < NB) atomicAdd(&g[(size_t)part(p) * NB + r], (unsigned long long)c);
        else if (r == NB) atomicAdd(&g[(size_t)Pg * (2 * NB + 2) + part(p)], (unsigned long long)c);
        else if (r < ROW_V + NB) atomicAdd(&g[(size_t)(Pg + part(p)) * NB + (r - ROW_V)], (unsigned long long)c);
    }
    __device__ __forceinline__ void sum_add(int which , int p, uint32_t v) const {
        if (SMEM) {
            const uint32_t a = sbase + 4u * (uint32_t)((ROW_KSUM + 2 * which) * P + p);
            red_shared_add(a, v & 0xffffu);
            red_shared_add_nz(a + 4u * (uint32_t)P, v >> 16);
        } else if (v) atomicAdd(&g[(size_t)Pg * (2 * NB + which) + part(p)], (unsigned long long)v);
    }
    __device__ __forceinline__ void buckets(int p, int kl, int vl) const {
        const int kb = (int)bfind_u32((uint32_t)kl) + 1;
        const int vb = (int)bfind_u32((uint32_t)vl) + 1;
        if (SMEM) {
            const uint32_t P4 = 4u * (uint32_t)P, pa = sbase + 4u * (uint32_t)p;
            red_shared_add(pa + (uint32_t)kb * P4, 1u);
            red_shared_add(pa + (uint32_t)(ROW_V + vb) * P4, 1u);
        } else {
            row_add(kb, p, 1u);
            row_add(ROW_V + vb, p, 1u);
        }
    }
    __device__ __forceinline__ void sums(int p, int kl, int vl) const {
        if (SMEM) {
            const uint32_t P4 = 4u * (uint32_t)P, pa = sbase + 4u * (uint32_t)p;
            const uint32_t ks = (uint32_t)max(kl, 0), vs = (uint32_t)max(vl, 0);
            red_shared_add(pa + ROW_KSUM * P4, ks & 0xffffu);
            red_shared_add_nz(pa + (ROW_KSUM + 1) * P4, ks >> 16);
            red_shared_add(pa + ROW_VSUM * P4, vs & 0xffffu);
            red_shared_add_nz(pa + (ROW_VSUM + 1) * P4, vs >> 16);
        } else {
            sum_add(0, p, (uint32_t)max(kl, 0));
            sum_add(1, p, (uint32_t)max(vl, 0));
        }
    }
    __device__ __forceinline__ void record(int p, int kl, int vl) const {
        buckets(p, kl, vl);
        sums(p, kl, vl);
    }
    __device__ __forceinline__ void record_rows(const int (&p)[ROWS], const int (&kl)[ROWS], const int (&vl)[ROWS]) const {
        if (SMEM) {
            uint32_t ks[ROWS], vs[ROWS], any = 0;
#pragma unroll
            for (int k = 0; k < ROWS; k++) {
                ks[k] = (uint32_t)max(kl[k], 0);
                vs[k] = (uint32_t)max(vl[k], 0);
                any |= ks[k] | vs[k];
                buckets(p[k], kl[k], vl[k]);
            }
            if (any < 0x10000u) {
                const uint32_t P4 = 4u * (uint32_t)P;
#pragma unroll
                for (int k = 0; k < ROWS; k++) {
                    const uint32_t pa = sbase + 4u * (uint32_t)p[k];
                    red_shared_add(pa + ROW_KSUM * P4, ks[k]);
                    red_shared_add(pa + ROW_VSUM * P4, vs[k]);
                }
            } else {
#pragma unroll
                for (int k = 0; k < ROWS; k++) sums(p[k], kl[k], vl[k]);
            }
        } else {
#pragma unroll
            for (int k = 0; k < ROWS; k++) record(p[k], kl[k], vl[k]);
        }
    }
    __device__ __noinline__ void fold_sums(int lane, uint32_t threshold) const {
        if constexpr (SMEM) {
            for (int i = lane; i < 2 * P; i += 32) {
                const int which = i >= P, p = which ? i - P : i;
                uint32_t *lo = &s[(ROW_KSUM + 2 * which) * P + p];
                if (*(volatile uint32_t *)lo >= threshold || *(volatile uint32_t *)(lo + P) >= threshold) {
                    const unsigned long long v = (unsigned long long)atomicExch(lo, 0u) +
                                                 ((unsigned long long)atomicExch(lo + P, 0u) << 16);
                    if (v) atomicAdd(&g[(size_t)Pg * (2 * NB + which) + part(p)], v);
                }
            }
        }
    }
};

constexpr unsigned long long ALIVE_EMPTY = ~0ull;
constexpr uint32_t ALIVE_FIELD_MAX = 0x7ffffffeu;
constexpr int ALIVE_MAX_PROBES = 96;

__device__ __forceinline__ uint64_t l2_policy_evict_last() {
    uint64_t pol;
    asm volatile("createpolicy.fractional.L2::evict_last.b64 %0, 1.0;" : "=l"(pol));
    return pol;
}
__device__ __forceinline__ uint64_t l2_policy_evict_first() {
    uint64_t pol;
    asm volatile("createpolicy.fractional.L2::evict_first.b64 %0, 1.0;" : "=l"(pol));
    return pol;
}
__device__ __forceinline__ ulonglong2 alive_ld_pair(const unsigned long long *p, uint64_t pol) {
    ulonglong2 v;
    asm volatile("ld.global.cg.L2::cache_hint.v2.u64 {%0, %1}, [%2], %3;" : "=l"(v.x), "=l"(v.y) : "l"(p), "l"(pol));
    return v;
}

__host__ __device__ __forceinline__ uint32_t alive_home(uint32_t x , uint32_t npairs) {
#ifdef __CUDA_ARCH__
    return __umulhi(x, npairs);
#else
    return (uint32_t)(((uint64_t)x * npairs) >> 32);
#endif
}

struct AliveTable {
    unsigned long long *slots;
    uint32_t npairs;
    uint32_t *status;
    uint64_t pol;
};

__device__ __forceinline__ void alive_red_max(unsigned long long *p, unsigned long long v, uint64_t pol) {
    asm volatile("red.global.max.L2::cache_hint.u64 [%0], %1, %2;" ::"l"(p), "l"(v), "l"(pol) : "memory");
}

__device__ __forceinline__ bool alive_probe_pair(const AliveTable t, uint32_t pair, uint32_t hash, uint32_t low, uint32_t &newest) {
    const unsigned long long stamp = ((unsigned long long)hash << 32) | low;
    unsigned long long *slot = t.slots + 2 * (size_t)pair;
    const ulonglong2 e = alive_ld_pair(slot, t.pol);
    newest = low;
#pragma unroll
    for (int s = 0; s < 2; s++) {
        unsigned long long v = s ? e.y : e.x;
        if (v == ALIVE_EMPTY) {
            v = atomicCAS(slot + s, ALIVE_EMPTY, stamp);
            if (v == ALIVE_EMPTY) return true;
        }
        if ((uint32_t)(v >> 32) == hash) {
            if (v >= stamp) newest = (uint32_t)v;
            else alive_red_max(slot + s, stamp, t.pol);
            return true;
        }
    }
    return false;
}

__device__ __noinline__ uint32_t alive_stamp_slow(const AliveTable t, uint32_t pair, uint32_t hash, uint32_t low) {
    uint32_t newest;
    for (int probe = 0; probe < ALIVE_MAX_PROBES; probe++) {
        if (alive_probe_pair(t, pair, hash, low, newest)) return newest;
        pair = pair + 1 == t.npairs ? 0 : pair + 1;
    }
    if (__ldcg(t.status + 2)) {
        for (uint32_t probe = ALIVE_MAX_PROBES; probe < t.npairs; probe++) {
            if (alive_probe_pair(t, pair, hash, low, newest)) return newest;
            pair = pair + 1 == t.npairs ? 0 : pair + 1;
        }
    }
    atomicAdd(t.status, 1u);
    return low;
}

__device__ __forceinline__ uint32_t alive_stamp(const AliveTable t, uint32_t pair, const ulonglong2 e, uint32_t hash, uint32_t low) {
    const bool hx = (uint32_t)(e.x >> 32) == hash, hy = (uint32_t)(e.y >> 32) == hash;
    const uint32_t seen = hx ? (uint32_t)e.x : (uint32_t)e.y;
    if ((hx || hy) && seen + 1u > low) return seen;
    unsigned long long *slot = t.slots + 2 * (size_t)pair;
    const unsigned long long stamp = ((unsigned long long)hash << 32) | low;
    const bool ex = e.x == ALIVE_EMPTY, ey = e.y == ALIVE_EMPTY;
    if ((hx && !ex) || (!hx && hy && !ey)) {
        alive_red_max(slot + (hx ? 0 : 1), stamp, t.pol);
        return low;
    }
    if (ex || ey) {
        unsigned long long *sl = slot + (ex ? 0 : 1);
        const unsigned long long old = atomicCAS(sl, ALIVE_EMPTY, stamp);
        if (old == ALIVE_EMPTY) return low;
        if ((uint32_t)(old >> 32) == hash) {
            if (old >= stamp) return (uint32_t)old;
            alive_red_max(sl, stamp, t.pol);
            return low;
        }
    }
    return alive_stamp_slow(t, pair, hash, low);
}

constexpr int ALIVE_CACHE_SET_BITS = 23, ALIVE_CACHE_TAG_BITS = 32 - ALIVE_CACHE_SET_BITS, ALIVE_CACHE_WAVE_BITS = 16 - ALIVE_CACHE_TAG_BITS;
constexpr uint32_t ALIVE_CACHE_WAVES = (1u << ALIVE_CACHE_WAVE_BITS) - 1;
static_assert(ALIVE_CACHE_TAG_BITS == 9 && ALIVE_CACHE_WAVE_BITS == 7, "16-bit ways");
__device__ __forceinline__ uint32_t alive_cache_ld(const uint32_t *p, uint64_t pol) {
    uint32_t v;
    asm volatile("ld.global.cg.L2::cache_hint.u32 %0, [%1], %2;" : "=r"(v) : "l"(p), "l"(pol));
    return v;
}
__device__ __forceinline__ bool alive_cache_newer(uint32_t c, uint32_t x, uint32_t wv) {
    const uint32_t tag = x & ((1u << ALIVE_CACHE_TAG_BITS) - 1u);
    const uint32_t w0 = c & 0xffffu, w1 = c >> 16;
    const uint32_t lo = (tag << ALIVE_CACHE_WAVE_BITS) | wv;
    return (w0 - lo - 1u < ALIVE_CACHE_WAVES - wv) || (w1 - lo - 1u < ALIVE_CACHE_WAVES - wv);
}
__device__ __forceinline__ void alive_cache_put(uint32_t *cache, uint32_t c, uint32_t x, uint32_t wv, uint32_t pick) {
    const uint32_t tag = x & ((1u << ALIVE_CACHE_TAG_BITS) - 1u);
    const uint32_t mine = (tag << ALIVE_CACHE_WAVE_BITS) | wv;
    const uint32_t w0 = c & 0xffffu, w1 = c >> 16;
    int way;
    if ((w0 >> ALIVE_CACHE_WAVE_BITS) == tag && w0) way = w0 >= mine ? -1 : 0;
    else if ((w1 >> ALIVE_CACHE_WAVE_BITS) == tag && w1) way = w1 >= mine ? -1 : 1;
    else way = w0 == 0 ? 0 : w1 == 0 ? 1 : (int)(pick & 1u);
    if (way >= 0) reinterpret_cast<unsigned short *>(cache + (x >> ALIVE_CACHE_TAG_BITS))[way] = (unsigned short)mine;
}

__device__ __forceinline__ bool alive_insert_unique(unsigned long long *slots, uint32_t npairs, unsigned long long entry) {
    uint32_t pair = alive_home((uint32_t)(entry >> 32), npairs);
    for (uint32_t probe = 0; probe < npairs; probe++) {
        unsigned long long *slot = slots + 2 * (size_t)pair;
#pragma unroll
        for (int s = 0; s < 2; s++)
            if (__ldcg(slot + s) == ALIVE_EMPTY && atomicCAS(slot + s, ALIVE_EMPTY, entry) == ALIVE_EMPTY) return true;
        pair = pair + 1 == npairs ? 0 : pair + 1;
    }
    return false;
}

__device__ __noinline__ void wide_tile_hashes(const int32_t *key_len, int64_t n, const uint8_t *tile_keys, int64_t tile,
                                              uint32_t *out , int lane) {
    uint64_t carry = 0;
    for (int k = 0; k < ROWS; k++) {
        const int64_t r = tile * TILE + 32 * k + lane;
        const int kl = r < n ? key_len[r] : -1;
        const uint64_t v = (uint64_t)max(kl, 0);
        uint64_t inc = v;
        for (int d = 1; d < 32; d <<= 1) {
            const uint64_t t = __shfl_up_sync(0xffffffffu, inc, d);
            if (lane >= d) inc += t;
        }
        out[32 * k + lane] = kl >= 0 ? fnv_global(tile_keys + carry + inc - v, kl) : 0u;
        carry += __shfl_sync(0xffffffffu, inc, 31);
    }
    __syncwarp();
}

struct AliveWaves {
    uint32_t *cache;
    uint32_t base;
    int shift;
};
__device__ __forceinline__ uint32_t alive_wave(uint32_t field, const AliveWaves w) {
    const uint32_t d = field - w.base;
    return (int32_t)d < 0 ? 0u : 1u + min(d >> w.shift, ALIVE_CACHE_WAVES - 1u);
}

struct TileDesc {
    uint32_t bits;
    __device__ __forceinline__ bool keys_staged() const { return bits & 1u; }
    __device__ __forceinline__ uint32_t key_lead() const { return (bits >> 1) & 15u; }
    __device__ __forceinline__ bool hdr_staged() const { return bits & 32u; }
};

template <int MODE>
struct TilePipe {
    const ScanParams &prm;
    unsigned char *wsm;
    uint32_t mbar, stage0;
    uint32_t keybuf, stage_bytes;
    int S, ntiles, tile0, gstride, lane;
    uint64_t pol;
    uint32_t phase = 0;
    int issued = 0;
    uint32_t infos = 0;
    uint64_t cur_g0 = 0, cur_g1 = 0, nxt_g0 = 0, nxt_g1 = 0;

    __device__ __forceinline__ int phys(int t) const { return MODE == MODE_EXACT ? ntiles - 1 - t : t; }
    __device__ __forceinline__ uint32_t stage(int b) const { return stage0 + (uint32_t)b * stage_bytes; }
    __device__ __forceinline__ unsigned char *stage_ptr(int b) const { return wsm + 128 + (size_t)b * stage_bytes; }

    __device__ __forceinline__ void copy(uint32_t dst, const void *src, uint32_t bytes, uint32_t bar) const {
        if (MODE == MODE_EXACT) bulk_g2s(dst, src, bytes, bar, pol);
        else bulk_g2s(dst, src, bytes, bar);
    }
    __device__ __forceinline__ uint32_t issue(int tile, int b, uint64_t g0, uint64_t g1) const {
        const uint32_t a = (uint32_t)g0 & 15u;
        const bool ok = (g1 - g0) - 1ull < (uint64_t)(keybuf - (uint32_t)KEYBUF_SLACK - a) && g1 <= prm.stage_limit;
        const bool hdr = prm.hdr_stage && (int64_t)(tile + 1) * TILE <= prm.n;
        const uint32_t kbytes = ok ? ((uint32_t)(g1 - g0) + a + 15u) & ~15u : 0u;
        const uint32_t bar = mbar + 8u * (uint32_t)b, dst = stage0 + (uint32_t)b * stage_bytes;
        if (ok || hdr) mbar_arrive_expect_tx(bar, kbytes + (hdr ? (uint32_t)HDR_BYTES : 0u));
        if (ok) copy(dst, prm.key_bytes + (g0 - a), kbytes, bar);
        if (hdr) {
            const int64_t r0 = (int64_t)tile * TILE;
            copy(dst + keybuf + HDR_P, prm.partition + r0, TILE * 4, bar);
            copy(dst + keybuf + HDR_TS, prm.ts_ms + r0, TILE * 8, bar);
            copy(dst + keybuf + HDR_KL, prm.key_len + r0, TILE * 4, bar);
            copy(dst + keybuf + HDR_VL, prm.value_len + r0, TILE * 4, bar);
        }
        return (ok ? 1u : 0u) | (a << 1) | (hdr ? 32u : 0u);
    }
    __device__ __forceinline__ void ring_load(int round, uint64_t &g0, uint64_t &g1) const {
        const int64_t t = tile0 + ((int64_t)round * 32 + lane) * gstride;
        if (t < ntiles) {
            const int pt = phys((int)t);
            g0 = __ldg(prm.key_tile_base + pt);
            g1 = __ldg(prm.key_tile_base + pt + 1);
        }
    }
    __device__ __forceinline__ void issue_next(int b) {
        if ((issued & 31) == 0 && issued) {
            cur_g0 = nxt_g0;
            cur_g1 = nxt_g1;
            ring_load((issued >> 5) + 1, nxt_g0, nxt_g1);
        }
        const uint64_t g0 = __shfl_sync(0xffffffffu, cur_g0, issued & 31), g1 = __shfl_sync(0xffffffffu, cur_g1, issued & 31);
        if (lane == 0) {
            const uint32_t d = issue(phys(tile0 + issued * gstride), b, g0, g1);
            infos = (infos & ~(0xffu << (8 * b))) | (d << (8 * b));
        }
        issued++;
    }
    __device__ __forceinline__ void start() {
        ring_load(0, cur_g0, cur_g1);
        ring_load(1, nxt_g0, nxt_g1);
        for (int b = 0; b < S - 1 && tile0 + b * gstride < ntiles; b++) issue_next(b);
    }
    __device__ __forceinline__ TileDesc next(int tile, int buf) {
        const TileDesc d{(__shfl_sync(0xffffffffu, infos, 0) >> (8 * buf)) & 0xffu};
        if (tile < ntiles - (S - 1) * gstride) issue_next(buf == 0 ? S - 1 : buf - 1);
        return d;
    }
    __device__ __forceinline__ void wait(int b) {
        mbar_wait(mbar + 8u * b, (phase >> b) & 1u);
        phase ^= 1u << b;
    }
};

struct TileRows {
    int p[ROWS], kl[ROWS], vl[ROWS];
    long long ts[ROWS];
    bool valid[ROWS];
    bool use[ROWS];
    bool clean;
};

struct WarpTotals {
    long long tmin = INT64_MAX, tmax = INT64_MIN;
    uint32_t smin = 0xffffffffu, smax = 0;
    uint32_t bad = 0;
    bool try_uni = true;
};

template <bool FULL, int MODE>
__device__ __forceinline__ void load_headers(const ScanParams &prm, TilePipe<MODE> &pipe, int buf, TileDesc d, int64_t rbase,
                                             int lane, TileRows &rec) {
    if (MODE != MODE_COUNTERS && d.hdr_staged()) {
        pipe.wait(buf);
        const uint32_t st = pipe.stage(buf);
#pragma unroll
        for (int k = 0; k < ROWS; k++) {
            const uint32_t r = 32u * k + lane;
            rec.valid[k] = true;
            rec.p[k] = (int)lds32(st + pipe.keybuf + HDR_P + 4u * r);
            rec.ts[k] = lds64(st + pipe.keybuf + HDR_TS + 8u * r);
            rec.kl[k] = (int)lds32(st + pipe.keybuf + HDR_KL + 4u * r);
            rec.vl[k] = (int)lds32(st + pipe.keybuf + HDR_VL + 4u * r);
        }
    } else {
#pragma unroll
        for (int k = 0; k < ROWS; k++) {
            const int64_t r = rbase + 32 * k;
            rec.valid[k] = FULL || r < prm.n;
            if (rec.valid[k]) {
                if (MODE == MODE_EXACT) {
                    rec.p[k] = ld_stream_s32(prm.partition + r, pipe.pol);
                    rec.ts[k] = ld_stream_s64(prm.ts_ms + r, pipe.pol);
                    rec.kl[k] = ld_stream_s32(prm.key_len + r, pipe.pol);
                    rec.vl[k] = ld_stream_s32(prm.value_len + r, pipe.pol);
                } else {
                    rec.p[k] = ld_stream_s32(prm.partition + r);
                    rec.ts[k] = ld_stream_s64(prm.ts_ms + r);
                    rec.kl[k] = ld_stream_s32(prm.key_len + r);
                    rec.vl[k] = ld_stream_s32(prm.value_len + r);
                }
            } else {
                rec.p[k] = 0; rec.ts[k] = INT64_MAX; rec.kl[k] = -1; rec.vl[k] = -1;
            }
        }
    }
}

template <bool FULL, bool SHARD>
__device__ __forceinline__ void partition_check(const ScanParams &prm, TileRows &rec) {
    bool inrange = true;
#pragma unroll
    for (int k = 0; k < ROWS; k++) {
        bool ok = (unsigned)rec.p[k] < (unsigned)prm.P;
        if (SHARD) {
            const int c = (int)__umulhi((uint32_t)rec.p[k], prm.shard_magic);
            ok = ok && rec.p[k] - c * prm.shard_world == prm.shard_rank;
            rec.p[k] = ok ? c : 0;
        }
        rec.use[k] = rec.valid[k] && ok;
        inrange = inrange && ok;
    }
    rec.clean = FULL && __all_sync(0xffffffffu, inrange);
}

template <bool SMEM>
__device__ __forceinline__ void count_tile(const Counters<SMEM> C, const TileRows &rec, bool count_it, int lane, WarpTotals &w) {
    const unsigned full = 0xffffffffu;
    if (!count_it) {
    } else if (rec.clean) {
        if (w.try_uni) {
            const int p0t = __shfl_sync(full, rec.p[0], 0);
            uint32_t kv4 = 0, vv4 = 0, big = 0;
            bool one = true;
#pragma unroll
            for (int k = 0; k < ROWS; k++) {
                const uint32_t kv = (uint32_t)max(rec.kl[k], 0), vv = (uint32_t)max(rec.vl[k], 0);
                one = one && rec.p[k] == p0t;
                kv4 += kv; vv4 += vv; big |= kv | vv;
            }
            if (__all_sync(full, one && big < (1u << 24))) {
#pragma unroll
                for (int k = 0; k < ROWS; k++) C.buckets(p0t, rec.kl[k], rec.vl[k]);
                const uint32_t ks = __reduce_add_sync(full, kv4);
                const uint32_t vs = __reduce_add_sync(full, vv4);
                if (lane == 0) {
                    C.sum_add(0, p0t, ks);
                    C.sum_add(1, p0t, vs);
                }
            } else {
            bool any_uni = false;
#pragma unroll
            for (int k = 0; k < ROWS; k++) {
                C.buckets(rec.p[k], rec.kl[k], rec.vl[k]);
                const int p0 = __shfl_sync(full, rec.p[k], 0);
                const unsigned m0 = __ballot_sync(full, rec.p[k] == p0);
                const bool small_row = __all_sync(full, (rec.kl[k] | rec.vl[k]) < (1 << 26));
                const uint32_t kv = (uint32_t)max(rec.kl[k], 0), vv = (uint32_t)max(rec.vl[k], 0);
                if (m0 == full && small_row) {
                    const uint32_t ks = __reduce_add_sync(full, kv);
                    const uint32_t vs = __reduce_add_sync(full, vv);
                    if (lane == 0) {
                        C.sum_add(0, p0, ks);
                        C.sum_add(1, p0, vs);
                    }
                    any_uni = true;
                } else {
                    const int l1 = __ffs(~m0) - 1;
                    const int p1 = __shfl_sync(full, rec.p[k], l1 & 31);
                    const unsigned m1 = __ballot_sync(full, rec.p[k] == p1);
                    if (small_row && (m0 | m1) == full) {
                        const bool in0 = (m0 >> lane) & 1u;
                        const uint32_t ks0 = __reduce_add_sync(full, in0 ? kv : 0u), vs0 = __reduce_add_sync(full, in0 ? vv : 0u);
                        const uint32_t ks1 = __reduce_add_sync(full, in0 ? 0u : kv), vs1 = __reduce_add_sync(full, in0 ? 0u : vv);
                        if (lane == 0) {
                            C.sum_add(0, p0, ks0);
                            C.sum_add(1, p0, vs0);
                        } else if (lane == l1) {
                            C.sum_add(0, p1, ks1);
                            C.sum_add(1, p1, vs1);
                        }
                        any_uni = true;
                    } else {
                        C.sums(rec.p[k], rec.kl[k], rec.vl[k]);
                    }
                }
            }
            w.try_uni = any_uni;
            }
        } else {
            C.record_rows(rec.p, rec.kl, rec.vl);
        }
    } else {
#pragma unroll
        for (int k = 0; k < ROWS; k++) {
            if (rec.use[k]) C.record(rec.p[k], rec.kl[k], rec.vl[k]);
            else if (rec.valid[k]) w.bad++;
        }
    }
    bool ts_fast = false;
    if (rec.clean && count_it) {
        const uint32_t hw = hi32(w.tmin);
        uint32_t x = hi32(w.tmax) ^ hw;
#pragma unroll
        for (int k = 0; k < ROWS; k++) x |= hi32(rec.ts[k]) ^ hw;
        ts_fast = x == 0;
    }
    if (ts_fast) {
        const uint32_t hw = hi32(w.tmin);
        const uint32_t l0 = (uint32_t)rec.ts[0], l1 = (uint32_t)rec.ts[1], l2 = (uint32_t)rec.ts[2], l3 = (uint32_t)rec.ts[3];
        const uint32_t lo = min(min(min(l0, l1), l2), min(l3, (uint32_t)w.tmin));
        const uint32_t hi = max(max(max(l0, l1), l2), max(l3, (uint32_t)w.tmax));
        w.tmin = pack64(lo, hw);
        w.tmax = pack64(hi, hw);
    } else if (count_it) {
        asm volatile("");
#pragma unroll
        for (int k = 0; k < ROWS; k++) {
            const bool u = rec.clean || rec.use[k];
            const long long t0 = u ? rec.ts[k] : INT64_MAX, t1 = u ? rec.ts[k] : INT64_MIN;
            w.tmin = t0 < w.tmin ? t0 : w.tmin;
            w.tmax = t1 > w.tmax ? t1 : w.tmax;
        }
    }
    if (count_it) {
#pragma unroll
        for (int k = 0; k < ROWS; k++) {
            const uint32_t sz = (uint32_t)max(rec.kl[k], 0) + (uint32_t)rec.vl[k];
            if (rec.vl[k] >= 0 && (rec.clean || rec.use[k])) {
                w.smin = min(w.smin, sz);
                w.smax = max(w.smax, sz);
            }
        }
    }
}

struct KeyOffsets {
    uint32_t off[ROWS];
    bool fixL;
    bool small;
    bool fix16;
};

__device__ __forceinline__ KeyOffsets key_offsets(const int (&kl)[ROWS], int lane) {
    const unsigned full = 0xffffffffu;
    const unsigned lt_mask = (1u << lane) - 1u;
    KeyOffsets o;
    const int lmax = max(max(kl[0], kl[1]), max(kl[2], kl[3]));
    const uint32_t lmin = min(min((uint32_t)kl[0], (uint32_t)kl[1]), min((uint32_t)kl[2], (uint32_t)kl[3]));
    static_assert(ROWS == 4, "written out for four rows");
    const int L = __reduce_max_sync(full, lmax);
    o.fixL = __reduce_min_sync(full, lmin) == (uint32_t)L && L < (1 << 16);
    o.small = L < (1 << 20);
    o.fix16 = o.fixL && L == 16;
    if (o.fixL) {
        const uint32_t Lu = (uint32_t)max(L, 0);
        if (!__any_sync(full, (kl[0] | kl[1] | kl[2] | kl[3]) < 0)) {
#pragma unroll
            for (int k = 0; k < ROWS; k++) o.off[k] = Lu * (uint32_t)(32 * k + lane);
        } else {
            uint32_t before = 0;
#pragma unroll
            for (int k = 0; k < ROWS; k++) {
                const unsigned m = __ballot_sync(full, kl[k] >= 0);
                o.off[k] = Lu * (before + __popc(m & lt_mask));
                before += __popc(m);
            }
        }
    } else {
        static_assert(ROWS == 4, "the packed scan below handles exactly four rows");
        uint32_t mxl = 0;
#pragma unroll
        for (int k = 0; k < ROWS; k++) mxl = max(mxl, (uint32_t)max(kl[k], 0));
        if (__all_sync(full, mxl < 2048u)) {
            const uint32_t v0 = (uint32_t)max(kl[0], 0), v1 = (uint32_t)max(kl[1], 0);
            const uint32_t v2 = (uint32_t)max(kl[2], 0), v3 = (uint32_t)max(kl[3], 0);
            uint32_t a = v0 | (v1 << 16), b = v2 | (v3 << 16);
#pragma unroll
            for (int d = 1; d < 32; d <<= 1) {
                const uint32_t ta = __shfl_up_sync(full, a, d), tb = __shfl_up_sync(full, b, d);
                if (lane >= d) { a += ta; b += tb; }
            }
            const uint32_t ea = __shfl_sync(full, a, 31), eb = __shfl_sync(full, b, 31);
            const uint32_t t0 = ea & 0xffffu, t1 = ea >> 16, t2 = eb & 0xffffu;
            o.off[0] = (a & 0xffffu) - v0;
            o.off[1] = t0 + (a >> 16) - v1;
            o.off[2] = t0 + t1 + (b & 0xffffu) - v2;
            o.off[3] = t0 + t1 + t2 + (b >> 16) - v3;
        } else if (o.small) {
            uint32_t c32 = 0;
#pragma unroll
            for (int k = 0; k < ROWS; k++) {
                const uint32_t v = (uint32_t)max(kl[k], 0);
                uint32_t inc = v;
#pragma unroll
                for (int d = 1; d < 32; d <<= 1) {
                    const uint32_t t = __shfl_up_sync(full, inc, d);
                    if (lane >= d) inc += t;
                }
                o.off[k] = c32 + inc - v;
                c32 += __shfl_sync(full, inc, 31);
            }
        }
    }
    return o;
}

template <bool CAPTURE, int MODE>
__device__ __forceinline__ void hash_tile(const ScanParams &prm, TilePipe<MODE> &pipe, int buf, TileDesc d, int tile, int64_t rbase,
                                          const TileRows &rec, const KeyOffsets &o, int lane, uint32_t (&h)[ROWS]) {
    const uint32_t kb = pipe.stage(buf);
    if (d.keys_staged()) {
        const uint32_t a0 = d.key_lead();
        if (!d.hdr_staged()) pipe.wait(buf);
        if (o.fix16 && a0 == 0) {
#pragma unroll
            for (int k = 0; k < ROWS; k += 2) {
                const uint4 qa = lds128(kb + o.off[k]);
                const uint4 qb = lds128(kb + o.off[k + 1]);
                uint32_t ha = FNV_BASIS, hb = FNV_BASIS;
                ha = fnv_word(ha, qa.x); hb = fnv_word(hb, qb.x);
                ha = fnv_word(ha, qa.y); hb = fnv_word(hb, qb.y);
                ha = fnv_word(ha, qa.z); hb = fnv_word(hb, qb.z);
                ha = fnv_word(ha, qa.w); hb = fnv_word(hb, qb.w);
                h[k] = ha;
                h[k + 1] = hb;
            }
        } else {
#pragma unroll
            for (int k = 0; k < ROWS; k++) h[k] = rec.kl[k] >= 0 ? fnv_smem(kb, a0 + o.off[k], rec.kl[k]) : 0u;
        }
    } else if (o.fixL || o.small) {
        const uint64_t g0 = prm.key_tile_base[tile];
#pragma unroll
        for (int k = 0; k < ROWS; k++)
            h[k] = (rec.valid[k] && rec.kl[k] >= 0) ? fnv_global(prm.key_bytes + g0 + o.off[k], rec.kl[k]) : 0u;
    } else {
        uint32_t *scratch = reinterpret_cast<uint32_t *>(pipe.stage_ptr(buf));
        wide_tile_hashes(prm.key_len, prm.n, prm.key_bytes + prm.key_tile_base[tile], tile, scratch, lane);
#pragma unroll
        for (int k = 0; k < ROWS; k++) h[k] = scratch[32 * k + lane];
    }
    if (CAPTURE) {
#pragma unroll
        for (int k = 0; k < ROWS; k++)
            if (rec.valid[k]) prm.hash_out[rbase + 32 * k] = rec.kl[k] >= 0 ? h[k] : 0u;
    }
}

struct ExactProbe {
    uint32_t x[ROWS];
    uint32_t low[ROWS];
    uint32_t cw[ROWS];
    bool live[ROWS];
};

__device__ __forceinline__ ExactProbe exact_probe(const ScanParams &prm, const AliveTable &AT, const AliveWaves &AW,
                                                  const TileRows &rec, const uint32_t (&h)[ROWS], int64_t rbase) {
    const bool cached = AW.cache != nullptr;
    const uint32_t r32 = (uint32_t)rbase;
    ExactProbe e;
#pragma unroll
    for (int k = 0; k < ROWS; k++) {
        e.live[k] = (rec.clean || rec.use[k]) && rec.kl[k] >= 0;
        uint32_t field;
        if (prm.seq) {
            const uint64_t f = e.live[k] ? ld_stream_u64(prm.seq + rbase + 32 * k) - prm.alive_origin + 1ull : 1ull;
            if (f - 1ull >= (uint64_t)ALIVE_FIELD_MAX) {
                atomicAdd(prm.alive_status + 1, 1u);
                e.live[k] = false;
            }
            field = (uint32_t)f;
        } else {
            field = (uint32_t)prm.alive_fbase + r32 + 32u * k;
        }
        e.low[k] = (field << 1) | (rec.vl[k] >= 0 ? 1u : 0u);
        e.x[k] = hll_mix(h[k]);
        e.cw[k] = 0;
        if (cached && e.live[k]) e.cw[k] = alive_cache_ld(AW.cache + (e.x[k] >> ALIVE_CACHE_TAG_BITS), AT.pol);
    }
    return e;
}

__device__ __forceinline__ void exact_resolve(const AliveTable &AT, const AliveWaves &AW, const ExactProbe &e, unsigned char *stage,
                                              int lane, unsigned lt_mask) {
    static_assert(TILE * 16 <= KEYBUF_MIN, "the queue stays inside the key part of the stage");
    uint4 *queue = reinterpret_cast<uint4 *>(stage);
    const bool cached = AW.cache != nullptr;
    __syncwarp();
    uint32_t qn = 0;
#pragma unroll
    for (int k = 0; k < ROWS; k++) {
        const bool go = e.live[k] && !(cached && alive_cache_newer(e.cw[k], e.x[k], alive_wave(e.low[k] >> 1, AW)));
        const unsigned m = __ballot_sync(0xffffffffu, go);
        if (go) queue[qn + __popc(m & lt_mask)] = make_uint4(e.x[k], e.low[k], e.cw[k], 0u);
        qn += __popc(m);
    }
    __syncwarp();
    for (uint32_t q0 = 0; q0 < qn; q0 += 32) {
        if (q0 + lane < qn) {
            const uint4 item = queue[q0 + lane];
            const uint32_t pr = alive_home(item.x, AT.npairs);
            const ulonglong2 en = alive_ld_pair(AT.slots + 2 * (size_t)pr, AT.pol);
            const uint32_t newest = alive_stamp(AT, pr, en, item.x, item.y);
            if (cached)
                alive_cache_put(AW.cache, item.z, item.x, max(alive_wave(item.y >> 1, AW), alive_wave(newest >> 1, AW)), newest >> 1);
        }
    }
    asm volatile("fence.proxy.async.shared::cta;" ::: "memory");
    __syncwarp();
}

__device__ __forceinline__ void sketch_tile(const ScanParams &prm, uint32_t floor_reg, const TileRows &rec, const uint32_t (&h)[ROWS]) {
    const uint32_t skip_mask = hll_skip_mask(prm.hll_p, floor_reg);
#pragma unroll
    for (int k = 0; k < ROWS; k++) {
        const uint32_t x = hll_mix(h[k]);
        if (((x & skip_mask) | (uint32_t)((rec.kl[k] | rec.vl[k]) >> 31)) == 0 && (rec.clean || rec.use[k])) hll_raise(prm.hll, prm.hll_p, x);
    }
}

template <bool SMEM>
__device__ __forceinline__ void flush_counters(const ScanParams &prm, const Counters<SMEM> &C, int tid, int warp, int lane) {
    const int nh = (ROW_V + NB) * C.P;
    for (int i = tid; i < nh; i += blockDim.x) {
        const uint32_t v = C.s[i];
        if (v) {
            const int row = i / C.P, pp = C.part(i - row * C.P);
            if (row < NB) atomicAdd(&prm.sums[(size_t)pp * NB + row], (unsigned long long)v);
            else if (row == NB) atomicAdd(&prm.sums[(size_t)prm.P * (2 * NB + 2) + pp], (unsigned long long)v);
            else atomicAdd(&prm.sums[(size_t)(prm.P + pp) * NB + (row - ROW_V)], (unsigned long long)v);
        }
    }
    if (warp == 0) C.fold_sums(lane, 1u);
}

__device__ __forceinline__ void flush_totals(const ScanParams &prm, WarpTotals w, unsigned char *wsm, size_t warp_bytes, int tid,
                                             int lane, int nwarps) {
    const unsigned full = 0xffffffffu;
    long long smin64 = w.smin != 0xffffffffu ? (long long)w.smin : INT64_MAX;
    long long smax64 = w.smin != 0xffffffffu ? (long long)w.smax : -1;
#pragma unroll
    for (int d = 16; d; d >>= 1) {
        const long long a = __shfl_xor_sync(full, w.tmin, d), b = __shfl_xor_sync(full, w.tmax, d);
        const long long c = __shfl_xor_sync(full, smin64, d), e = __shfl_xor_sync(full, smax64, d);
        w.tmin = a < w.tmin ? a : w.tmin;
        w.tmax = b > w.tmax ? b : w.tmax;
        smin64 = c < smin64 ? c : smin64;
        smax64 = e > smax64 ? e : smax64;
        w.bad += __shfl_xor_sync(full, w.bad, d);
    }
    long long *red = reinterpret_cast<long long *>(wsm + 64);
    if (lane == 0) {
        red[0] = w.tmin; red[1] = w.tmax; red[2] = smin64; red[3] = smax64;
        if (w.bad) atomicAdd(&prm.sums[sums_words(prm.P) - 1], (unsigned long long)w.bad);
    }
    __syncthreads();
    if (tid == 0) {
        for (int i = 1; i < nwarps; i++) {
            const long long *rw = reinterpret_cast<const long long *>(wsm + (size_t)i * warp_bytes + 64);
            w.tmin = rw[0] < w.tmin ? rw[0] : w.tmin;
            w.tmax = rw[1] > w.tmax ? rw[1] : w.tmax;
            smin64 = rw[2] < smin64 ? rw[2] : smin64;
            smax64 = rw[3] > smax64 ? rw[3] : smax64;
        }
        if (w.tmin != INT64_MAX) {
            atomicMin(&prm.minmax[0], w.tmin);
            atomicMax(&prm.minmax[1], w.tmax);
        }
        if (smax64 >= 0) {
            atomicMin(reinterpret_cast<unsigned long long *>(&prm.minmax[2]), (unsigned long long)smin64);
            atomicMax(reinterpret_cast<unsigned long long *>(&prm.minmax[3]), (unsigned long long)smax64);
        }
    }
}

template <int MODE, bool SMEM, bool CAPTURE, bool SHARD = false>
__global__ void __launch_bounds__(MODE == MODE_COUNTERS ? MAX_THREADS : HASH_MAX_THREADS, 1) scan_kernel(const ScanParams prm) {
    constexpr bool HASH = MODE != MODE_COUNTERS;
    extern __shared__ __align__(128) unsigned char smem_raw[];
    const int tid = threadIdx.x, lane = tid & 31, warp = tid >> 5, nwarps = blockDim.x >> 5;
    const unsigned lt_mask = (1u << lane) - 1u;
    const int P = SHARD ? prm.Pc : prm.P;
    uint32_t *scnt = reinterpret_cast<uint32_t *>(smem_raw);
    const size_t cta_bytes = SMEM ? smem_counter_bytes(P) : CTA_SCRATCH;
    const uint32_t KEYBUF = (uint32_t)prm.keybuf;
    const int S = HASH ? prm.stages : 0;
    const size_t warp_bytes = warp_smem_bytes(HASH, prm.keybuf, S, prm.hdr_stage);
    unsigned char *wsm = smem_raw + cta_bytes + (size_t)warp * warp_bytes;
    const uint32_t mbar = smem_u32(wsm);
    const uint32_t stage0 = smem_u32(wsm) + 128;
    const Counters<SMEM> C{smem_u32(scnt), scnt, prm.sums, P, prm.P, SHARD ? prm.shard_world : 1, SHARD ? prm.shard_rank : 0};
    const uint64_t pol_stream = MODE == MODE_EXACT ? l2_policy_evict_first() : 0;
    const AliveTable AT{prm.alive_table, prm.alive_pairs, prm.alive_status, MODE == MODE_EXACT ? l2_policy_evict_last() : 0};
    const AliveWaves AW{prm.alive_cache, prm.alive_wave_base, prm.alive_wave_shift};
    const bool count_it = !(MODE == MODE_EXACT && prm.alive_only);

    if (SMEM) {
        const int nw = P * SMEM_ROWS;
        for (int i = tid; i < nw; i += blockDim.x) scnt[i] = 0;
    }
    if (HASH && lane == 0) {
        for (int b = 0; b < S; b++) mbar_init(mbar + 8u * b, 1);
        fence_mbar_init();
    }
    __syncthreads();

    WarpTotals tot;
    uint32_t floor_reg = MODE == MODE_HLL ? ld_cg_u32(prm.hll_floor) : 0u;

    const int ntiles = (int)prm.ntiles;
    const int gstride = (int)gridDim.x * nwarps;
    int tile = (int)blockIdx.x * nwarps + warp;
    TilePipe<MODE> pipe{prm, wsm, mbar, stage0, KEYBUF, KEYBUF + (prm.hdr_stage ? (uint32_t)HDR_BYTES : 0u), S, ntiles, tile, gstride, lane,
                        pol_stream};
    if (HASH) pipe.start();

    auto scan_tile = [&](auto full_tag, int tile, int buf, TileDesc d) {
        constexpr bool FULL = decltype(full_tag)::value;
        const int64_t rbase = (int64_t)tile * TILE + lane;
        TileRows rec;
        load_headers<FULL>(prm, pipe, buf, d, rbase, lane, rec);
        partition_check<FULL, SHARD>(prm, rec);
        uint32_t h[ROWS] = {0u, 0u, 0u, 0u};
        if (MODE != MODE_EXACT) count_tile(C, rec, count_it, lane, tot);
        if (HASH) hash_tile<CAPTURE>(prm, pipe, buf, d, tile, rbase, rec, key_offsets(rec.kl, lane), lane, h);
        if (MODE == MODE_EXACT) {
            unsigned char *queue = pipe.stage_ptr(buf);
            const ExactProbe e = exact_probe(prm, AT, AW, rec, h, rbase);
            count_tile(C, rec, count_it, lane, tot);
            exact_resolve(AT, AW, e, queue, lane, lt_mask);
        }
        if (MODE == MODE_HLL) sketch_tile(prm, floor_reg, rec, h);
    };

    int buf = 0;
    for (int it = 0; tile < ntiles; tile += gstride, ++it) {
        const TileDesc d = HASH ? pipe.next(tile, buf) : TileDesc{0u};
        const int pt = pipe.phys(tile);
        if ((int64_t)(pt + 1) * TILE <= prm.n) scan_tile(std::true_type{}, pt, buf, d);
        else scan_tile(std::false_type{}, pt, buf, d);
        if (HASH) buf = buf + 1 == S ? 0 : buf + 1;
        if (SMEM && (it & (FOLD_TILES - 1)) == FOLD_TILES - 1) C.fold_sums(lane, 1u << 30);
        tot.try_uni = tot.try_uni || (it & 15) == 15;
        if (MODE == MODE_HLL) {
            if (((it & 3) == 3 && ((it >> 2) & 31) == (warp & 31)) || (it < 2 && warp == it + 1))
                hll_refresh_slice(prm.hll, prm.hll_p, prm.hll_floor, (blockIdx.x + (uint32_t)(it >> 2) * 37u) & (HLL_SLICES - 1), lane);
            if (it < 4 || (it & 15) == 15) floor_reg = ld_cg_u32(prm.hll_floor);
        }
    }

    __syncthreads();
    if (SMEM) flush_counters(prm, C, tid, warp, lane);
    flush_totals(prm, tot, wsm, warp_bytes, tid, lane, nwarps);
}

__global__ void __launch_bounds__(256) tile_key_bytes_kernel(const int32_t *key_len, int64_t n, int64_t ntiles,
                                                             uint64_t *tile_base ) {
    const int lane = threadIdx.x & 31;
    const int64_t gw = ((int64_t)blockIdx.x * blockDim.x + threadIdx.x) >> 5, gs = ((int64_t)gridDim.x * blockDim.x) >> 5;
    for (int64_t tile = gw; tile < ntiles; tile += gs) {
        uint64_t s = 0;
#pragma unroll
        for (int k = 0; k < ROWS; k++) {
            const int64_t r = tile * TILE + k * 32 + lane;
            if (r < n) {
                const int32_t v = key_len[r];
                s += v > 0 ? (uint64_t)v : 0;
            }
        }
#pragma unroll
        for (int d = 16; d; d >>= 1) s += __shfl_xor_sync(0xffffffffu, s, d);
        if (lane == 0) tile_base[tile + 1] = s;
    }
    if (blockIdx.x == 0 && threadIdx.x == 0) tile_base[0] = 0;
}

__global__ void __launch_bounds__(1024) tile_base_scan_kernel(uint64_t *tile_base, int64_t ntiles) {
    __shared__ uint64_t wsum[32];
    __shared__ uint64_t carry_s;
    const int tid = threadIdx.x, lane = tid & 31, warp = tid >> 5;
    if (tid == 0) carry_s = 0;
    __syncthreads();
    for (int64_t base = 1; base <= ntiles; base += 1024) {
        const int64_t i = base + tid;
        const uint64_t v = i <= ntiles ? tile_base[i] : 0;
        uint64_t inc = v;
#pragma unroll
        for (int d = 1; d < 32; d <<= 1) {
            const uint64_t t = __shfl_up_sync(0xffffffffu, inc, d);
            if (lane >= d) inc += t;
        }
        if (lane == 31) wsum[warp] = inc;
        __syncthreads();
        uint64_t wb = 0;
        for (int w = 0; w < warp; w++) wb += wsum[w];
        const uint64_t out = carry_s + wb + inc;
        if (i <= ntiles) tile_base[i] = out;
        __syncthreads();
        if (tid == 1023) carry_s = out;
        __syncthreads();
    }
}

constexpr int THREADS = 256;
__global__ void __launch_bounds__(THREADS) alive_hll_kernel(const unsigned long long *table, size_t nslots, uint32_t *hll, int hll_p) {
    const size_t stride = (size_t)gridDim.x * THREADS;
    for (size_t i = (size_t)blockIdx.x * THREADS + threadIdx.x; i < nslots; i += stride) {
        const unsigned long long v = table[i];
        if (v != ALIVE_EMPTY && (v & 1ull)) hll_raise(hll, hll_p, (uint32_t)(v >> 32));
    }
}

__global__ void __launch_bounds__(THREADS) alive_export_kernel(const unsigned long long *table, size_t nslots, uint64_t origin, int mode,
                                                               unsigned long long *counter, uint32_t *out_hash,
                                                               unsigned long long *out_stamp, unsigned long long cap) {
    const int lane = threadIdx.x & 31;
    const size_t stride = (size_t)gridDim.x * THREADS;
    const size_t rounds = (nslots + stride - 1) / stride;
    for (size_t it = 0; it < rounds; it++) {
        const size_t i = it * stride + (size_t)blockIdx.x * THREADS + threadIdx.x;
        const unsigned long long v = i < nslots ? table[i] : ALIVE_EMPTY;
        const bool live = v != ALIVE_EMPTY;
        const unsigned m = __ballot_sync(0xffffffffu, live);
        if (!m) continue;
        unsigned long long base = 0;
        if (lane == 0) base = atomicAdd(counter, (unsigned long long)__popc(m));
        base = __shfl_sync(0xffffffffu, base, 0);
        if (mode == 1 && live) {
            const unsigned long long slot = base + __popc(m & ((1u << lane) - 1u));
            if (slot < cap) {
                const unsigned long long field = (v >> 1) & 0x7fffffffull;
                out_hash[slot] = hll_unmix((uint32_t)(v >> 32));
                out_stamp[slot] = ((origin + field) << 1) | (v & 1ull);
            }
        }
    }
}

__global__ void __launch_bounds__(THREADS) alive_import_kernel(const AliveTable t, uint64_t origin, const uint32_t *hash,
                                                               const unsigned long long *stamp, int64_t count) {
    AliveTable tt = t;
    tt.pol = l2_policy_evict_last();
    const int64_t stride = (int64_t)gridDim.x * THREADS;
    for (int64_t i = (int64_t)blockIdx.x * THREADS + threadIdx.x; i < count; i += stride) {
        const unsigned long long st = stamp[i];
        const unsigned long long field = (st >> 1) - origin;
        if (field - 1ull >= (unsigned long long)ALIVE_FIELD_MAX) {
            atomicAdd(t.status + 1, 1u);
            continue;
        }
        const uint32_t x = hll_mix(hash[i]);
        alive_stamp_slow(tt, alive_home(x, t.npairs), x, ((uint32_t)field << 1) | (uint32_t)(st & 1ull));
    }
}

__global__ void __launch_bounds__(THREADS) alive_count_kernel(const unsigned long long *table, size_t nslots, unsigned long long *out) {
    const size_t stride = (size_t)gridDim.x * THREADS;
    unsigned alive = 0, occ = 0;
    for (size_t i = (size_t)blockIdx.x * THREADS + threadIdx.x; i < nslots; i += stride) {
        const unsigned long long v = table[i];
        occ += v != ALIVE_EMPTY;
        alive += v != ALIVE_EMPTY && (v & 1ull);
    }
    alive = __reduce_add_sync(0xffffffffu, alive);
    occ = __reduce_add_sync(0xffffffffu, occ);
    if ((threadIdx.x & 31) == 0) {
        if (alive) atomicAdd(out, (unsigned long long)alive);
        if (occ) atomicAdd(out + 2, (unsigned long long)occ);
    }
}

__global__ void __launch_bounds__(THREADS) alive_rehash_kernel(const unsigned long long *old_slots, size_t old_nslots,
                                                               unsigned long long *new_slots, uint32_t new_npairs, uint32_t *status) {
    const size_t stride = (size_t)gridDim.x * THREADS;
    for (size_t i = (size_t)blockIdx.x * THREADS + threadIdx.x; i < old_nslots; i += stride) {
        const unsigned long long v = old_slots[i];
        if (v != ALIVE_EMPTY && !alive_insert_unique(new_slots, new_npairs, v)) atomicAdd(status, 1u);
    }
}

__global__ void __launch_bounds__(THREADS) alive_rebase_kernel(unsigned long long *slots, size_t nslots) {
    const size_t stride = (size_t)gridDim.x * THREADS;
    for (size_t i = (size_t)blockIdx.x * THREADS + threadIdx.x; i < nslots; i += stride) {
        const unsigned long long v = slots[i];
        if (v != ALIVE_EMPTY) slots[i] = v & 0xffffffff00000001ull;
    }
}

__global__ void state_init_kernel(unsigned long long *sums, size_t nsums, long long *minmax, uint32_t *hll, size_t nhll,
                                  uint32_t *hll_floor) {
    const size_t stride = (size_t)gridDim.x * blockDim.x;
    for (size_t i = (size_t)blockIdx.x * blockDim.x + threadIdx.x; i < nsums; i += stride) sums[i] = 0;
    for (size_t i = (size_t)blockIdx.x * blockDim.x + threadIdx.x; i < nhll; i += stride) hll[i] = 0;
    if (blockIdx.x == 0 && threadIdx.x == 0) {
        minmax[0] = INT64_MAX;
        minmax[1] = INT64_MIN;
        reinterpret_cast<unsigned long long *>(minmax)[2] = ~0ull;
        reinterpret_cast<unsigned long long *>(minmax)[3] = 0ull;
        for (int i = 0; i <= HLL_SLICES; i++) hll_floor[i] = 0;
    }
}

__global__ void fnv32_kernel(int64_t n, const int32_t *key_len, const uint64_t *key_off, const uint8_t *key_bytes,
                             uint32_t *out) {
    for (int64_t i = (int64_t)blockIdx.x * blockDim.x + threadIdx.x; i < n; i += (int64_t)gridDim.x * blockDim.x)
        out[i] = key_len[i] < 0 ? 0u : fnv_global(key_bytes + key_off[i], key_len[i]);
}

__global__ void merge_export_kernel(const unsigned long long *sums, size_t nsums, const long long *minmax,
                                    const uint32_t *hll, size_t nhll, int rank, int world, unsigned long long *buf) {
    const size_t stride = (size_t)gridDim.x * blockDim.x, t0 = (size_t)blockIdx.x * blockDim.x + threadIdx.x;
    const size_t nmm = (size_t)world * 4, hw = nhll / 8, total = nsums + nmm + (size_t)world * hw;
    for (size_t i = t0; i < total; i += stride) {
        unsigned long long v = 0;
        if (i < nsums) v = sums[i];
        else if (i < nsums + nmm) {
            const size_t j = i - nsums;
            if ((int)(j / 4) == rank) v = (unsigned long long)minmax[j % 4];
        } else {
            const size_t j = i - nsums - nmm;
            if ((int)(j / hw) == rank) {
                const uint32_t *r = hll + (j % hw) * 8;
#pragma unroll
                for (int k = 0; k < 8; k++) v |= (unsigned long long)(r[k] & 0xffu) << (8 * k);
            }
        }
        buf[i] = v;
    }
}

__global__ void merge_import_kernel(unsigned long long *sums, size_t nsums, long long *minmax, uint32_t *hll,
                                    size_t nhll, uint32_t *hll_floor, int world, const unsigned long long *buf) {
    const size_t stride = (size_t)gridDim.x * blockDim.x, t0 = (size_t)blockIdx.x * blockDim.x + threadIdx.x;
    for (size_t i = t0; i < nsums; i += stride) sums[i] = buf[i];
    const unsigned long long *mm = buf + nsums;
    const size_t hw = nhll / 8;
    const unsigned long long *hb = mm + (size_t)world * 4;
    for (size_t i = t0; i < nhll; i += stride) {
        uint32_t m = 0;
        for (int r = 0; r < world; r++) m = max(m, (uint32_t)(hb[(size_t)r * hw + i / 8] >> (8 * (i % 8))) & 0xffu);
        hll[i] = m;
    }
    if (t0 == 0) {
        long long tmin = INT64_MAX, tmax = INT64_MIN;
        unsigned long long smin = ~0ull, smax = 0;
        for (int r = 0; r < world; r++) {
            tmin = min(tmin, (long long)mm[r * 4 + 0]);
            tmax = max(tmax, (long long)mm[r * 4 + 1]);
            smin = min(smin, mm[r * 4 + 2]);
            smax = max(smax, mm[r * 4 + 3]);
        }
        minmax[0] = tmin;
        minmax[1] = tmax;
        reinterpret_cast<unsigned long long *>(minmax)[2] = smin;
        reinterpret_cast<unsigned long long *>(minmax)[3] = smax;
        for (int i = 0; i <= HLL_SLICES; i++) hll_floor[i] = 0;
    }
}

}
```

Measured before the change: 83.80 billion.

## Overlap back-to-back scan launches with programmatic dependent launch

Consecutive non-exact scan kernels are now launched with programmatic stream serialization, so the next grid can start its prologue (shared-memory counter init, mbarrier setup) while the previous one is flushing. The kernel waits on griddepcontrol.wait before touching global state and signals launch_dependents before its counter flush. Timing events now bracket a whole run of scans instead of each launch, and runs are closed before any non-scan work. Host result buffers also become pinned memory. This adds bookkeeping complexity and makes correctness depend on every non-scan path ending the run before it touches shared state.

```diff
diff --git a/kafka_topic_analyzer_b200/csrc/kta_api.cu b/kafka_topic_analyzer_b200/csrc/kta_api.cu
--- a/kafka_topic_analyzer_b200/csrc/kta_api.cu
+++ b/kafka_topic_analyzer_b200/csrc/kta_api.cu
@@ -126,9 +126,9 @@
     } pc;
     uint64_t next_seq = 0;
     bool finalized = false;
-    std::vector<uint64_t> h_sums;
-    long long h_minmax[4] = {0, 0, 0, 0};
-    std::vector<uint32_t> h_hll;
+    PinnedBuf<uint64_t> h_sums;
+    PinnedBuf<long long> h_minmax;
+    PinnedBuf<uint32_t> h_hll;
     uint64_t h_alive = 0;
     int shard_world = 1, shard_rank = 0;
     int columns = 0;
@@ -136,7 +136,12 @@
     size_t smem_optin = 0;
     uint64_t launches = 0, records = 0;
     bool timing = false;
-    std::vector<std::pair<cudaEvent_t, cudaEvent_t>> ev_pool;
+    bool scan_tail = false, run_open = false;
+    struct TimedRun {
+        cudaEvent_t start, end;
+        uint64_t scans;
+    };
+    std::vector<TimedRun> ev_pool;
     size_t ev_used = 0;
     double scan_ms = 0;
     uint64_t scan_launches_timed = 0;
@@ -145,6 +150,21 @@
 static int set_device(const kta_handle *h) {
     CU(cudaSetDevice(h->device));
     return KTA_OK;
+}
+
+static int scan_run_end(kta_handle *h) {
+    h->scan_tail = false;
+    if (h->run_open) {
+        CU(cudaEventRecord(h->ev_pool[h->ev_used - 1].end, h->stream));
+        h->run_open = false;
+    }
+    return KTA_OK;
+}
+
+static int begin(kta_handle *h) {
+    int rc;
+    if ((rc = set_device(h))) return rc;
+    return scan_run_end(h);
 }
 
 static bool keys_travel(const kta_handle *h) { return h->need_hash || h->d_hash_out || h->pt.ncounts; }
@@ -382,7 +402,7 @@
     AliveKeys &a = h->alive;
     if (!a.d_table) return fail(KTA_ERR_NOT_ENABLED, "count_alive_keys was not enabled");
     int rc;
-    if ((rc = set_device(h))) return rc;
+    if ((rc = begin(h))) return rc;
     if ((rc = ring_flush(h))) return rc;
     if ((rc = alive_settle(h))) return rc;
     if (a.rebased)
@@ -415,7 +435,7 @@
     if (!a.d_table) return fail(KTA_ERR_NOT_ENABLED, "count_alive_keys was not enabled");
     if (count == 0) return KTA_OK;
     int rc;
-    if ((rc = set_device(h))) return rc;
+    if ((rc = begin(h))) return rc;
     if ((rc = alive_settle(h))) return rc;
     const AlivePending p{ScanParams{}, 0, 0, -1, dev_hash, dev_stamp, count};
     if ((rc = alive_apply(h, p))) return rc;
@@ -438,7 +458,7 @@
     if (h->stream) cudaStreamSynchronize(h->stream);
     for (auto &c : h->chunks)
         if (c.free_ev) cudaEventDestroy(c.free_ev);
-    for (auto &e : h->ev_pool) { cudaEventDestroy(e.first); cudaEventDestroy(e.second); }
+    for (auto &e : h->ev_pool) { cudaEventDestroy(e.start); cudaEventDestroy(e.end); }
     cudaStream_t own = h->own_stream ? h->stream : nullptr;
     delete h;
     if (own) cudaStreamDestroy(own);
@@ -486,6 +506,9 @@
     if ((rc = h->d_sums.alloc((int64_t)h->nsums)) || (rc = h->d_minmax.alloc(4)) || (rc = h->d_hll_floor.alloc(HLL_SLICES + 2)))
         return rc;
     if (h->nhll && (rc = h->d_hll.alloc((int64_t)h->nhll))) return rc;
+    if ((rc = h->h_sums.alloc((int64_t)h->nsums)) || (rc = h->h_minmax.alloc(4)) || (h->nhll && (rc = h->h_hll.alloc((int64_t)h->nhll))))
+        return rc;
+    memset(h->h_minmax.get(), 0, 32);
     if (cfg->count_alive_keys == 1 && (rc = alive_create(h))) return rc;
     h->smem_optin = prop.sharedMemPerBlockOptin;
     if (cfg->shard_world > 1) {
@@ -535,7 +558,7 @@
 extern "C" int kta_set_stream(kta_handle *h, void *stream) {
     if (!h) return fail(KTA_ERR_INVALID, "null handle");
     int rc;
-    if ((rc = set_device(h))) return rc;
+    if ((rc = begin(h))) return rc;
     CU(cudaStreamSynchronize(h->stream));
     if (h->own_stream) CU(cudaStreamDestroy(h->stream));
     h->stream = (cudaStream_t)stream;
@@ -579,24 +602,43 @@
     prm.keybuf = keybuf;
     prm.stages = stages;
     const int grid = (int)std::min<int64_t>((prm.ntiles + threads / 32 - 1) / (threads / 32), h->sm_count);
+    const bool overlap = mode != MODE_EXACT && !capture;
+    int rc;
+    if (!overlap && (rc = scan_run_end(h))) return rc;
     if (prm.alive_cache) CU(cudaMemsetAsync(prm.alive_cache, 0, (size_t)4 << ALIVE_CACHE_SET_BITS, h->stream));
-    cudaEvent_t e0 = nullptr, e1 = nullptr;
-    if (h->timing) {
+    if (h->timing && !h->run_open) {
         if (h->ev_used == h->ev_pool.size()) {
             cudaEvent_t a, b;
             CU(cudaEventCreate(&a));
             CU(cudaEventCreate(&b));
-            h->ev_pool.emplace_back(a, b);
+            h->ev_pool.push_back({a, b, 0});
         }
-        e0 = h->ev_pool[h->ev_used].first;
-        e1 = h->ev_pool[h->ev_used].second;
+        h->ev_pool[h->ev_used].scans = 0;
+        CU(cudaEventRecord(h->ev_pool[h->ev_used].start, h->stream));
         h->ev_used++;
-        CU(cudaEventRecord(e0, h->stream));
-    }
-    SCAN_KERNELS[h->smem_counters][h->shard_world > 1][mode][capture]<<<grid, threads, sm, h->stream>>>(prm);
+        h->run_open = true;
+    }
+    const ScanFn fn = SCAN_KERNELS[h->smem_counters][h->shard_world > 1][mode][capture];
+    if (overlap && h->scan_tail) {
+        cudaLaunchAttribute attr[1];
+        attr[0].id = cudaLaunchAttributeProgrammaticStreamSerialization;
+        attr[0].val.programmaticStreamSerializationAllowed = 1;
+        cudaLaunchConfig_t lc = {};
+        lc.gridDim = dim3((unsigned)grid);
+        lc.blockDim = dim3((unsigned)threads);
+        lc.dynamicSmemBytes = sm;
+        lc.stream = h->stream;
+        lc.attrs = attr;
+        lc.numAttrs = 1;
+        CU(cudaLaunchKernelEx(&lc, fn, prm));
+    } else {
+        fn<<<grid, threads, sm, h->stream>>>(prm);
+    }
     CU(cudaGetLastError());
     h->launches++;
-    if (h->timing) CU(cudaEventRecord(e1, h->stream));
+    if (h->timing) h->ev_pool[h->ev_used - 1].scans++;
+    if (!overlap) return scan_run_end(h);
+    h->scan_tail = true;
     return KTA_OK;
 }
 
@@ -700,6 +742,7 @@
     }
     if (exact && (rc = alive_prepare(h, prm, seq_ends))) return rc;
     if ((rc = launch_scan_raw(h, prm, key_readable, key_bytes))) return rc;
+    if ((h->tl.buckets || h->pt.ncounts) && (rc = scan_run_end(h))) return rc;
     if (h->tl.buckets && (rc = launch_timeline(h, prm))) return rc;
     if (h->pt.ncounts && (rc = launch_partitioner(h, prm, key_bytes))) return rc;
     if (exact && (rc = alive_scanned(h, prm, key_readable, key_bytes, chunk))) return rc;
@@ -709,13 +752,15 @@
 }
 
 static int collect_timing(kta_handle *h) {
-    for (size_t i = 0; i < h->ev_used; i++) {
+    const size_t done = h->run_open ? h->ev_used - 1 : h->ev_used;
+    for (size_t i = 0; i < done; i++) {
         float ms = 0;
-        CU(cudaEventElapsedTime(&ms, h->ev_pool[i].first, h->ev_pool[i].second));
+        CU(cudaEventElapsedTime(&ms, h->ev_pool[i].start, h->ev_pool[i].end));
         h->scan_ms += ms;
-        h->scan_launches_timed++;
-    }
-    h->ev_used = 0;
+        h->scan_launches_timed += h->ev_pool[i].scans;
+    }
+    if (h->run_open && done) std::swap(h->ev_pool[0], h->ev_pool[done]);
+    h->ev_used -= done;
     return KTA_OK;
 }
 
@@ -723,7 +768,11 @@
     return LogEnv{h->stream, h->sm_count, h->smem_optin, h->cfg.num_partitions, h->d_tb_scratch, h->launches};
 }
 
-static int derive_tile_base(kta_handle *h, const int32_t *d_klen, int64_t n) { return log_tile_base(log_env(h), d_klen, n); }
+static int derive_tile_base(kta_handle *h, const int32_t *d_klen, int64_t n) {
+    int rc;
+    if ((rc = scan_run_end(h))) return rc;
+    return log_tile_base(log_env(h), d_klen, n);
+}
 
 static ScanParams scan_params(int64_t n, uint64_t seq_base, const int32_t *partition, const int64_t *ts_ms, const int32_t *key_len,
                               const int32_t *value_len, const uint8_t *key_bytes, const uint64_t *key_tile_base, const uint64_t *seq) {
@@ -763,6 +812,7 @@
     if (h->pt.ncounts && !b->key_bytes) {
         if (b->key_bytes_len > 0) return fail(KTA_ERR_INVALID, "key_bytes is NULL but key_bytes_len is %lld", (long long)b->key_bytes_len);
         uint64_t total = 0;
+        if ((rc = scan_run_end(h))) return rc;
         CU(cudaMemcpyAsync(&total, prm.key_tile_base + (b->n + TILE - 1) / TILE, 8, cudaMemcpyDeviceToHost, h->stream));
         CU(cudaStreamSynchronize(h->stream));
         if (total) return fail(KTA_ERR_INVALID, "key_bytes is NULL but the batch has %llu key bytes (the partitioner check hashes them)",
@@ -789,7 +839,7 @@
     if (records_out) *records_out = 0;
     if (nbatches == 0) return KTA_OK;
     int rc;
-    if ((rc = set_device(h))) return rc;
+    if ((rc = begin(h))) return rc;
     if ((rc = ring_flush(h))) return rc;
     if ((rc = alive_settle_if_any(h))) return rc;
     LogScan &L = h->log;
@@ -859,7 +909,7 @@
     }
     if (offs.empty()) return KTA_OK;
     int rc;
-    if ((rc = set_device(h))) return rc;
+    if ((rc = begin(h))) return rc;
     cudaStream_t s = h->stream;
     LogScan &L = h->log;
     const int64_t nb = (int64_t)offs.size();
@@ -899,7 +949,7 @@
     }
     if (add.empty()) return KTA_OK;
     int rc;
-    if ((rc = set_device(h))) return rc;
+    if ((rc = begin(h))) return rc;
     return log_add_txn_ranges(h->log, log_env(h), add);
 }
 
@@ -998,6 +1048,7 @@
                            const uint64_t *seq_ends = nullptr) {
     int rc;
     if ((rc = launch_scan(h, prm, key_readable, key_bytes, h->cur, seq_ends))) return rc;
+    if ((rc = scan_run_end(h))) return rc;
     CU(cudaEventRecord(h->chunks[h->cur].free_ev, h->stream));
     h->cur = (h->cur + 1) % NCHUNK;
     return KTA_OK;
@@ -1010,6 +1061,8 @@
 
 static int ring_flush(kta_handle *h) {
     if (h->pc.n == 0) return KTA_OK;
+    int rc;
+    if ((rc = scan_run_end(h))) return rc;
     Chunk &c = h->chunks[h->cur];
     const int64_t n = h->pc.n, kb = h->pc.kb;
     const int64_t ntiles = (n + TILE - 1) / TILE;
@@ -1024,7 +1077,6 @@
         CU(cudaMemcpyAsync(c.d_tile_base, c.h_tile_base, (ntiles + 1) * 8, cudaMemcpyHostToDevice, s));
     }
     const ScanParams prm = scan_params(n, h->next_seq, c.d_partition, c.d_ts, c.d_klen, c.d_vlen, c.d_keys, c.d_tile_base, nullptr);
-    int rc;
     if ((rc = ring_scan_chunk(h, prm, (kb + 15) & ~(int64_t)15, kb))) return rc;
     h->next_seq += (uint64_t)n;
     push_cursor_bind(h);
@@ -1033,7 +1085,7 @@
 
 static int __attribute__((noinline)) push_slow(kta_handle *h, int64_t kl) {
     int rc;
-    if ((rc = set_device(h))) return rc;
+    if ((rc = begin(h))) return rc;
     if (!h->ring_host_ready) {
         if ((rc = ring_host_init(h))) return rc;
         push_cursor_bind(h);
@@ -1087,7 +1139,7 @@
         for (int64_t i = 0; i < b->n; i++)
             if (b->key_len[i] > 0) return fail(KTA_ERR_INVALID, "key_bytes is NULL but record %lld has a %d-byte key (the partitioner "
                                                "check hashes it)", (long long)i, b->key_len[i]);
-    if ((rc = set_device(h))) return rc;
+    if ((rc = begin(h))) return rc;
     if ((rc = ring_flush(h))) return rc;
     if ((rc = ring_dev_init(h))) return rc;
     uint64_t seq_base = 0;
@@ -1164,7 +1216,7 @@
 extern "C" int kta_sync(kta_handle *h) {
     if (!h) return fail(KTA_ERR_INVALID, "null handle");
     int rc;
-    if ((rc = set_device(h))) return rc;
+    if ((rc = begin(h))) return rc;
     if ((rc = ring_flush(h))) return rc;
     CU(cudaStreamSynchronize(h->stream));
     if ((rc = alive_settle(h))) return rc;
@@ -1174,7 +1226,7 @@
 extern "C" int kta_reset(kta_handle *h) {
     if (!h) return fail(KTA_ERR_INVALID, "null handle");
     int rc;
-    if ((rc = set_device(h))) return rc;
+    if ((rc = begin(h))) return rc;
     h->pc.n = 0;
     h->pc.kb = 0;
     h->next_seq = 0;
@@ -1198,7 +1250,7 @@
 extern "C" int kta_finalize(kta_handle *h) {
     if (!h) return fail(KTA_ERR_INVALID, "null handle");
     int rc;
-    if ((rc = set_device(h))) return rc;
+    if ((rc = begin(h))) return rc;
     if ((rc = ring_flush(h))) return rc;
     cudaStream_t s = h->stream;
     if ((rc = alive_settle(h))) return rc;
@@ -1209,11 +1261,9 @@
         CU(cudaGetLastError());
         h->launches++;
     }
-    h->h_sums.resize(h->nsums);
-    h->h_hll.resize(h->nhll);
-    CU(cudaMemcpyAsync(h->h_sums.data(), h->d_sums, h->nsums * 8, cudaMemcpyDeviceToHost, s));
+    CU(cudaMemcpyAsync(h->h_sums, h->d_sums, h->nsums * 8, cudaMemcpyDeviceToHost, s));
     CU(cudaMemcpyAsync(h->h_minmax, h->d_minmax, 32, cudaMemcpyDeviceToHost, s));
-    if (h->nhll) CU(cudaMemcpyAsync(h->h_hll.data(), h->d_hll, h->nhll * 4, cudaMemcpyDeviceToHost, s));
+    if (h->nhll) CU(cudaMemcpyAsync(h->h_hll, h->d_hll, h->nhll * 4, cudaMemcpyDeviceToHost, s));
     if (h->tl.buckets) {
         h->tl.h_bins.resize(h->tl.words());
         CU(cudaMemcpyAsync(h->tl.h_bins.data(), h->tl.d_bins, h->tl.words() * 8, cudaMemcpyDeviceToHost, s));
@@ -1246,7 +1296,7 @@
 
 static uint64_t raw_counter(const kta_handle *h, int which, int32_t p) {
     const int P = h->cfg.num_partitions;
-    const uint64_t *s = h->h_sums.data();
+    const uint64_t *s = h->h_sums;
     uint64_t knn = 0, alive = 0;
     for (int b = 0; b < NB; b++) {
         knn += s[(size_t)p * NB + b];
@@ -1313,7 +1363,7 @@
     const int rc = check_read(h, 0, false);
     if (rc) return rc;
     const int P = h->cfg.num_partitions;
-    const unsigned long long *mm = reinterpret_cast<const unsigned long long *>(h->h_minmax);
+    const unsigned long long *mm = reinterpret_cast<const unsigned long long *>(h->h_minmax.get());
     switch (which) {
         case KTA_SMALLEST_MESSAGE: *out = mm[2] == ~0ull ? 0 : mm[2]; return KTA_OK;
         case KTA_LARGEST_MESSAGE: *out = mm[3]; return KTA_OK;
@@ -1395,7 +1445,7 @@
     if (buckets && bins > TL_MAX_BINS)
         return fail(KTA_ERR_INVALID, "timeline of %lld partitions x %d indices exceeds 2^24 bins", (long long)P, buckets + 2);
     int rc;
-    if ((rc = set_device(h))) return rc;
+    if ((rc = begin(h))) return rc;
     Timeline t;
     if (buckets) {
         if ((rc = t.d_bins.alloc(3 * bins))) return rc;
@@ -1460,7 +1510,7 @@
             if (counts[i] == counts[j]) return fail(KTA_ERR_INVALID, "partition count %d given twice", counts[j]);
     }
     int rc;
-    if ((rc = set_device(h))) return rc;
+    if ((rc = begin(h))) return rc;
     if (ncounts && !h->d_crc32_tables) {
         uint32_t tables[4][256];
         crc_slicing_tables_host(tables, ZLIB_CRC32_POLY);
@@ -1541,7 +1591,7 @@
     const int p = h->cfg.hll_precision, q = 32 - p;
     const double m = (double)h->nhll;
     std::vector<double> C((size_t)q + 2, 0.0);
-    for (uint32_t r : h->h_hll) C[std::min<uint32_t>(r, (uint32_t)q + 1)] += 1.0;
+    for (size_t i = 0; i < h->nhll; i++) C[std::min<uint32_t>(h->h_hll[i], (uint32_t)q + 1)] += 1.0;
     double z = m * hll_tau(1.0 - C[(size_t)q + 1] / m);
     for (int k = q; k >= 1; k--) z = 0.5 * (z + C[(size_t)k]);
     z += m * hll_sigma(C[0] / m);
@@ -1564,7 +1614,7 @@
     if (!h || n < 0 || (n && (!key_len || !out))) return fail(KTA_ERR_INVALID, "bad argument");
     if (n == 0) return KTA_OK;
     int rc;
-    if ((rc = set_device(h))) return rc;
+    if ((rc = begin(h))) return rc;
     std::vector<uint64_t> off((size_t)n);
     uint64_t acc = 0;
     for (int64_t i = 0; i < n; i++) {
@@ -1595,7 +1645,7 @@
     if (!h || n < 0 || (n && (!key_len || !murmur2 || !crc32))) return fail(KTA_ERR_INVALID, "bad argument");
     if (n == 0) return KTA_OK;
     int rc;
-    if ((rc = set_device(h))) return rc;
+    if ((rc = begin(h))) return rc;
     std::vector<uint64_t> off((size_t)n);
     uint64_t acc = 0;
     for (int64_t i = 0; i < n; i++) {
@@ -1632,7 +1682,7 @@
 extern "C" int kta_set_hash_capture(kta_handle *h, uint32_t *dev_out) {
     if (!h) return fail(KTA_ERR_INVALID, "null handle");
     int rc;
-    if ((rc = set_device(h))) return rc;
+    if ((rc = begin(h))) return rc;
     if ((rc = ring_flush(h))) return rc;
     h->d_hash_out = dev_out;
     h->pc.hash = keys_travel(h);
@@ -1649,7 +1699,7 @@
 extern "C" int kta_merge_export_device(kta_handle *h, int32_t rank, int32_t world, uint64_t *dev_buf) {
     if (!h || !dev_buf || world < 1 || rank < 0 || rank >= world) return fail(KTA_ERR_INVALID, "bad argument");
     int rc;
-    if ((rc = set_device(h))) return rc;
+    if ((rc = begin(h))) return rc;
     if ((rc = ring_flush(h))) return rc;
     if ((rc = alive_settle_if_any(h))) return rc;
     merge_export_kernel<<<h->sm_count, 256, 0, h->stream>>>(h->d_sums, h->nsums, h->d_minmax, h->d_hll, h->nhll, rank,
@@ -1671,7 +1721,7 @@
 extern "C" int kta_merge_import_device(kta_handle *h, int32_t world, const uint64_t *dev_buf) {
     if (!h || !dev_buf || world < 1) return fail(KTA_ERR_INVALID, "bad argument");
     int rc;
-    if ((rc = set_device(h))) return rc;
+    if ((rc = begin(h))) return rc;
     merge_import_kernel<<<h->sm_count, 256, 0, h->stream>>>(h->d_sums, h->nsums, h->d_minmax, h->d_hll, h->nhll,
                                                            h->d_hll_floor, world,
                                                            reinterpret_cast<const unsigned long long *>(dev_buf));
@@ -1698,7 +1748,7 @@
     if (!h) return fail(KTA_ERR_INVALID, "null handle");
     if (!h->alive.d_table) return fail(KTA_ERR_NOT_ENABLED, "count_alive_keys was not enabled");
     int rc;
-    if ((rc = set_device(h))) return rc;
+    if ((rc = begin(h))) return rc;
     if ((rc = ring_flush(h))) return rc;
     if ((rc = alive_settle(h))) return rc;
     if (slots) *slots = (uint64_t)h->alive.pairs * 2;
@@ -1710,6 +1760,8 @@
 
 extern "C" int kta_set_timing(kta_handle *h, int enabled) {
     if (!h) return fail(KTA_ERR_INVALID, "null handle");
+    int rc;
+    if ((rc = begin(h))) return rc;
     h->timing = enabled != 0;
     h->scan_ms = 0;
     h->scan_launches_timed = 0;
@@ -1719,7 +1771,7 @@
 extern "C" int kta_scan_time_ms(kta_handle *h, double *total_ms, uint64_t *launches) {
     if (!h) return fail(KTA_ERR_INVALID, "null handle");
     int rc;
-    if ((rc = set_device(h))) return rc;
+    if ((rc = begin(h))) return rc;
     CU(cudaStreamSynchronize(h->stream));
     if ((rc = collect_timing(h))) return rc;
     if (total_ms) *total_ms = h->scan_ms;
diff --git a/kafka_topic_analyzer_b200/csrc/kta_kernels.cuh b/kafka_topic_analyzer_b200/csrc/kta_kernels.cuh
--- a/kafka_topic_analyzer_b200/csrc/kta_kernels.cuh
+++ b/kafka_topic_analyzer_b200/csrc/kta_kernels.cuh
@@ -1077,6 +1077,7 @@
         fence_mbar_init();
     }
     __syncthreads();
+    if (MODE != MODE_EXACT) asm volatile("griddepcontrol.wait;" ::: "memory");
 
     WarpTotals tot;
     uint32_t floor_reg = MODE == MODE_HLL ? ld_cg_u32(prm.hll_floor) : 0u;
@@ -1123,6 +1124,7 @@
     }
 
     __syncthreads();
+    if (MODE != MODE_EXACT) asm volatile("griddepcontrol.launch_dependents;" ::: "memory");
     if (SMEM) flush_counters(prm, C, tid, warp, lane);
     flush_totals(prm, tot, wsm, warp_bytes, tid, lane, nwarps);
 }
```

New measurement: 85.33 billion, median of 6. 1.8% higher.
